# ChaissonLab/LRA

Hardware: AMD Instinct MI355X
Metric: aligned Gbp/s, 30 kb ONT vs GRCh38 (MapRead_lowacc end to end incl. SAM text), per job (higher is better)
Workload: dtype int32

## Files before the change

lra_amd/csrc/merge_extend.hip:

```cpp
#include "common.h"
#include "scan.h"
#include "std_sort.h"
#include <rocprim/rocprim.hpp>

namespace {

struct MeArgs {
  uint64_t n_slots; int numAln; int K;
  const uint32_t* nChains; const uint64_t* chainStart; const uint32_t* nSplit; const uint32_t* spStatus; const uint8_t* spStrand; const int32_t* spChrom;
  const uint64_t* matchOff; const uint32_t* mq; const uint32_t* mt; const uint32_t* box;
  const uint64_t* pos;
  uint32_t* nCl; uint32_t* nGr; const uint64_t* clBase; const uint64_t* grBase;
  uint64_t* cStart; uint64_t* cEnd; int* cStrand; int* cChrom; int* cRead; uint32_t* cGroup;
  uint32_t* gFirst; uint32_t* gLast; uint32_t* gSlot;
  const uint32_t* eCount; uint32_t* gSize; const uint64_t* anchorOff;
  const uint32_t* eq; const uint32_t* et; const int* el;
  uint32_t* aq; uint32_t* at; int32_t* alen; uint32_t* gbox; int32_t* gstrand; int32_t* gchrom; uint64_t* scratch;
};

template <int PASS>
__global__ void me_merge(MeArgs a) {
  const uint64_t s = (uint64_t)blockIdx.x * blockDim.x + threadIdx.x;
  if (s >= a.n_slots) return;
  const uint64_t r = s / a.numAln;
  uint32_t nsp = 0;
  if ((uint32_t)(s % a.numAln) < a.nChains[r] && !a.spStatus[s]) nsp = a.nSplit[s];
  if (PASS == 0) { a.nCl[s] = nsp; a.nGr[s] = 0; }
  if (nsp == 0) return;
  const uint64_t cs = a.chainStart[s];
  const uint64_t cb = PASS ? a.clBase[s] : 0, gb = PASS ? a.grBase[s] : 0;
  uint32_t g = 0, g0 = 0;
  for (uint32_t t = 0; t < nsp; t++) {
    const uint64_t x = cs + t;
    if (t > 0) {
      const uint64_t xp = x - 1;
      int qdist = 9999, tdist = 9999;
      if (a.spChrom[xp] == a.spChrom[x] && a.spStrand[xp] == a.spStrand[x]) {
        const uint32_t pqs = a.box[4 * xp], pts = a.box[4 * xp + 2], pte = a.box[4 * xp + 3];
        const uint32_t cqe = a.box[4 * x + 1], cts = a.box[4 * x + 2], cte = a.box[4 * x + 3];
        qdist = pqs > cqe ? (int)(pqs - cqe) : 0;
        if (a.spStrand[xp] == 0) tdist = pts >= cte ? (int)(pts - cte) : 9999;
        else tdist = pte <= cts ? (int)(cts - pte) : 9999;
      }
      if (!(qdist <= 500 && tdist <= 500)) {
        if (PASS) { a.gFirst[gb + g] = (uint32_t)(cb + g0); a.gLast[gb + g] = (uint32_t)(cb + t - 1); a.gSlot[gb + g] = (uint32_t)s; }
        g++; g0 = t;
      }
    }
    if (PASS) {
      const uint64_t c = cb + t;
      a.cStart[c] = a.matchOff[x]; a.cEnd[c] = a.matchOff[x + 1]; a.cStrand[c] = a.spStrand[x]; a.cChrom[c] = a.spChrom[x]; a.cRead[c] = (int)r;
      a.cGroup[c] = (uint32_t)(gb + g);
    }
  }
  if (PASS) { a.gFirst[gb + g] = (uint32_t)(cb + g0); a.gLast[gb + g] = (uint32_t)(cb + nsp - 1); a.gSlot[gb + g] = (uint32_t)s; }
  g++;
  if (PASS == 0) a.nGr[s] = g;
}

__global__ void __launch_bounds__(64) me_keys(uint64_t ncl, const uint64_t* __restrict__ cStart, const uint64_t* __restrict__ cEnd, const uint32_t* __restrict__ mq,
                                              const uint32_t* __restrict__ mt, uint64_t* key, uint32_t* val) {
  for (uint64_t c = blockIdx.x; c < ncl; c += gridDim.x)
    for (uint64_t i = cStart[c] + threadIdx.x; i < cEnd[c]; i += 64) {
      const uint32_t q = mq[i], t = mt[i];
      key[i] = ((uint64_t)((long long)q - (long long)t + (1LL << 32)) << 31) | q;
      val[i] = (uint32_t)i;
    }
}

__global__ void __launch_bounds__(64) me_gather_sorted(uint64_t ncl, const uint64_t* __restrict__ cStart, const uint64_t* __restrict__ cEnd, const int* __restrict__ cChrom,
                                                       const uint64_t* __restrict__ pos, const uint32_t* __restrict__ val, const uint32_t* __restrict__ mq,
                                                       const uint32_t* __restrict__ mt, uint32_t* sq, uint32_t* st) {
  for (uint64_t c = blockIdx.x; c < ncl; c += gridDim.x) {
    const uint32_t coff = (uint32_t)pos[cChrom[c]];
    for (uint64_t i = cStart[c] + threadIdx.x; i < cEnd[c]; i += 64) { const uint32_t v = val[i]; sq[i] = mq[v]; st[i] = mt[v] + coff; }
  }
}

__global__ void me_group_size(uint64_t ng, MeArgs a) {
  const uint64_t g = (uint64_t)blockIdx.x * blockDim.x + threadIdx.x;
  if (g >= ng) return;
  uint32_t n = 0;
  for (uint32_t c = a.gFirst[g]; c <= a.gLast[g]; c++) n += a.eCount[c];
  a.gSize[g] = n;
}

__global__ void __launch_bounds__(64) me_concat(uint64_t ng, MeArgs a) {
  const int lane = threadIdx.x;
  for (uint64_t g = blockIdx.x; g < ng; g += gridDim.x) {
    uint64_t o = a.anchorOff[g];
    uint32_t qS = 0xFFFFFFFFu, qE = 0, tS = 0xFFFFFFFFu, tE = 0;
    for (uint32_t c = a.gFirst[g]; c <= a.gLast[g]; c++) {
      const uint64_t b = a.cStart[c];
      const uint32_t n = a.eCount[c];
      const uint32_t coff = (uint32_t)a.pos[a.cChrom[c]];
      for (uint32_t i = lane; i < n; i += 64) {
        const uint32_t q = a.eq[b + i], t = a.et[b + i] - coff; const int l = a.el[b + i];
        a.aq[o + i] = q; a.at[o + i] = t; a.alen[o + i] = l;
        qS = min(qS, q); qE = max(qE, q + (uint32_t)l); tS = min(tS, t); tE = max(tE, t + (uint32_t)l);
      }
      o += n;
    }
    for (int off = 32; off > 0; off >>= 1) {
      qS = min(qS, (uint32_t)__shfl_xor(qS, off)); qE = max(qE, (uint32_t)__shfl_xor(qE, off));
      tS = min(tS, (uint32_t)__shfl_xor(tS, off)); tE = max(tE, (uint32_t)__shfl_xor(tE, off));
    }
    if (lane == 0) {
      const bool any = o > a.anchorOff[g];
      a.gbox[4 * g] = any ? qS : 0; a.gbox[4 * g + 1] = any ? qE : 0; a.gbox[4 * g + 2] = any ? tS : 0; a.gbox[4 * g + 3] = any ? tE : 0;
      a.gstrand[g] = any ? a.cStrand[a.gLast[g]] : 0; a.gchrom[g] = any ? a.cChrom[a.gLast[g]] : 0;
    }
  }
}

struct LongLess {
  const uint32_t* Q; const uint32_t* T; const int32_t* L; int strand;
  __device__ bool operator()(uint64_t i, uint64_t j) const {
    if (strand == 0) { if (Q[i] != Q[j]) return Q[i] < Q[j]; return T[i] < T[j]; }
    const uint32_t ei = Q[i] + (uint32_t)L[i], ej = Q[j] + (uint32_t)L[j];
    if (ei != ej) return ei > ej;
    return T[i] < T[j];
  }
};

__global__ void me_trim(uint64_t ng, const uint64_t* __restrict__ anchorOff, uint32_t* aq, uint32_t* at, int32_t* alen, const int32_t* __restrict__ gstrand,
                        uint64_t* scratch, int minLen) {
  const uint64_t g = (uint64_t)blockIdx.x * blockDim.x + threadIdx.x;
  if (g >= ng) return;
  const uint64_t b = anchorOff[g];
  const uint32_t n = (uint32_t)(anchorOff[g + 1] - b);
  uint32_t* Q = aq + b; uint32_t* T = at + b; int32_t* L = alen + b;
  uint64_t* idx = scratch + b;
  const int S = gstrand ? gstrand[g] : 0;
  uint32_t m = 0;
  for (uint32_t i = 0; i < n; i++) if (L[i] >= minLen) idx[m++] = i;
  LongLess lt{Q, T, L, S};
  lra_std_sort::std_sort(idx, (long)m, lt);
  for (uint32_t ln = 1; ln < m; ln++) {
    const uint32_t prev = (uint32_t)idx[ln - 1], cur = (uint32_t)idx[ln];
    int overlap_r = 0, overlap_g = 0;
    if (S == 0) {
      if (Q[cur] < Q[prev] + (uint32_t)L[prev] && Q[cur] >= Q[prev] + (uint32_t)L[prev] - 30u) overlap_r = (int)(Q[prev] + (uint32_t)L[prev] - Q[cur]);
    } else {
      if (Q[cur] + (uint32_t)L[cur] > Q[prev] && Q[cur] + (uint32_t)L[cur] <= Q[prev] + 30u) overlap_r = (int)(Q[cur] + (uint32_t)L[cur] - Q[prev]);
    }
    if (T[cur] < T[prev] + (uint32_t)L[prev] && T[cur] >= T[prev] + (uint32_t)L[prev] - 30u) overlap_g = (int)(T[prev] + (uint32_t)L[prev] - T[cur]);
    if (overlap_r > 0 || overlap_g > 0) {
      const int overlap = max(overlap_r, overlap_g);
      if (S == 1) Q[prev] += (uint32_t)(overlap + 1);
      L[prev] -= overlap + 1;
    }
  }
}

__global__ void me_iota(uint64_t n, uint64_t* out) {
  const uint64_t i = (uint64_t)blockIdx.x * blockDim.x + threadIdx.x;
  if (i <= n) out[i] = i;
}

__global__ void me_gather_off(uint64_t n, const uint64_t* idx, const uint64_t* src, uint64_t* out) {
  const uint64_t i = (uint64_t)blockIdx.x * blockDim.x + threadIdx.x;
  if (i <= n) out[i] = src[idx[i]];
}

inline size_t sz(size_t n, size_t e) { return (n * e + 255) / 256 * 256; }

}

extern "C" int lra_merge_extend_batch(lra_ctx* ctx, const lra_chain_result* ch, const lra_split_result* sp, const lra_btwn_result* bt, const char* d_seq,
                                      const uint64_t* d_read_off, const char* d_genome, const uint64_t* h_chrom_pos, int n_chrom, int K,
                                      lra_merge_result* out) {
  if (!ctx || !ch || !sp || !bt || !out || !h_chrom_pos || n_chrom < 1 || K < 1) return LRA_ERR_INVALID;
  memset(out, 0, sizeof *out);
  LRA_HIP_CHECK(ctx, hipSetDevice(ctx->device));
  hipStream_t st = ctx->stream;
  const uint64_t slots = sp->n_slots, NM = bt->n_matches;
  out->n_slots = slots;
  if (slots == 0) return LRA_OK;
  const size_t npos = (size_t)n_chrom + 1;
  auto take = [](char*& p, size_t n, size_t e) { char* r = p; p += sz(n, e); return r; };
  char* w = (char*)lra_ensure(ctx, 37, sz(slots + 2, 4) * 2 + sz(slots + 2, 8) * 2 + sz(npos, 8) + 4096);
  if (!w) return LRA_ERR_NOMEM;
  MeArgs a;
  memset(&a, 0, sizeof a);
  a.n_slots = slots; a.numAln = ch->num_aln; a.K = K; a.nChains = ch->d_n_chains; a.chainStart = ch->d_chain_start; a.nSplit = sp->d_n_split; a.spStatus = sp->d_status;
  a.spStrand = sp->d_sp_strand; a.spChrom = sp->d_sp_chrom; a.matchOff = bt->d_match_off; a.mq = bt->d_match_q; a.mt = bt->d_match_t; a.box = bt->d_box;
  a.nCl = (uint32_t*)take(w, slots + 2, 4); a.nGr = (uint32_t*)take(w, slots + 2, 4);
  uint64_t* clBase = (uint64_t*)take(w, slots + 2, 8); uint64_t* grBase = (uint64_t*)take(w, slots + 2, 8);
  uint64_t* dpos = (uint64_t*)take(w, npos, 8);
  a.clBase = clBase; a.grBase = grBase; a.pos = dpos;
  LRA_HIP_CHECK(ctx, hipMemcpyAsync(dpos, h_chrom_pos, npos * 8, hipMemcpyHostToDevice, st));
  const unsigned gs = (unsigned)((slots + 255) / 256);
  lra_time_begin(ctx, "merge_extend");
  hipLaunchKernelGGL(me_merge<0>, dim3(gs), dim3(256), 0, st, a);
  lra_time_end(ctx);
  { int rc = lra_exclusive_scan<uint32_t>(ctx, (long)slots, a.nCl, clBase); if (rc) return rc; }
  { int rc = lra_exclusive_scan<uint32_t>(ctx, (long)slots, a.nGr, grBase); if (rc) return rc; }
  uint64_t NCL = 0, NG = 0;
  LRA_HIP_CHECK(ctx, hipMemcpyAsync(&NCL, clBase + slots, 8, hipMemcpyDeviceToHost, st));
  LRA_HIP_CHECK(ctx, hipMemcpyAsync(&NG, grBase + slots, 8, hipMemcpyDeviceToHost, st));
  LRA_HIP_CHECK(ctx, hipStreamSynchronize(st));
  out->n_groups = NG; out->d_slot_group_off = grBase;
  char* wc = (char*)lra_ensure(ctx, 38, sz(NCL + 1, 8) * 2 + sz(NCL + 1, 4) * 5 + sz(4 * NCL + 4, 4) + sz(NG + 2, 4) * 6 + sz(4 * NG + 4, 4) + sz(NG + 2, 8) * 2 + 4096);
  char* wm = (char*)lra_ensure(ctx, 100, sz(NM + 1, 8) * 2 + sz(NM + 1, 4) * 6 + 4096);
  if (!wc || !wm) return LRA_ERR_NOMEM;
  a.cStart = (uint64_t*)take(wc, NCL + 1, 8); a.cEnd = (uint64_t*)take(wc, NCL + 1, 8);
  a.cStrand = (int*)take(wc, NCL + 1, 4); a.cChrom = (int*)take(wc, NCL + 1, 4); a.cRead = (int*)take(wc, NCL + 1, 4); a.cGroup = (uint32_t*)take(wc, NCL + 1, 4);
  uint32_t* eCount = (uint32_t*)take(wc, NCL + 1, 4); uint32_t* ebox = (uint32_t*)take(wc, 4 * NCL + 4, 4);
  a.gFirst = (uint32_t*)take(wc, NG + 2, 4); a.gLast = (uint32_t*)take(wc, NG + 2, 4); a.gSlot = (uint32_t*)take(wc, NG + 2, 4); a.gSize = (uint32_t*)take(wc, NG + 2, 4);
  a.gstrand = (int32_t*)take(wc, NG + 2, 4); a.gchrom = (int32_t*)take(wc, NG + 2, 4); a.gbox = (uint32_t*)take(wc, 4 * NG + 4, 4);
  uint64_t* anchorOff = (uint64_t*)take(wc, NG + 2, 8); uint64_t* iota = (uint64_t*)take(wc, NG + 2, 8);
  uint64_t* key = (uint64_t*)take(wm, NM + 1, 8); uint64_t* key2 = (uint64_t*)take(wm, NM + 1, 8);
  uint32_t* val = (uint32_t*)take(wm, NM + 1, 4); uint32_t* val2 = (uint32_t*)take(wm, NM + 1, 4); uint32_t* sq = (uint32_t*)take(wm, NM + 1, 4);
  uint32_t* stt = (uint32_t*)take(wm, NM + 1, 4); uint32_t* eq = (uint32_t*)take(wm, NM + 1, 4); uint32_t* et = (uint32_t*)take(wm, NM + 1, 4);
  int* el = (int*)key;
  a.eCount = eCount; a.eq = eq; a.et = et; a.el = el; a.anchorOff = anchorOff; a.scratch = key2;
  if (NCL == 0) { LRA_HIP_CHECK(ctx, hipMemsetAsync(anchorOff, 0, 16, st)); LRA_HIP_CHECK(ctx, hipStreamSynchronize(st)); out->d_anchor_off = anchorOff; return LRA_OK; }
  lra_time_begin(ctx, "merge_extend");
  hipLaunchKernelGGL(me_merge<1>, dim3(gs), dim3(256), 0, st, a);
  lra_time_end(ctx);
  const unsigned gw = (unsigned)std::min<uint64_t>(NCL, (uint64_t)ctx->num_cu * 32);
  if (NM > 0) {
    lra_time_begin(ctx, "merge_extend");
    hipLaunchKernelGGL(me_keys, dim3(gw), dim3(64), 0, st, NCL, (const uint64_t*)a.cStart, (const uint64_t*)a.cEnd, a.mq, a.mt, key, val);
    const int rc = lra_segsort_pairs_scratch(ctx, key, key2, val, val2, NM, NCL, a.cStart, a.cEnd, 0, 64);
    if (rc) { lra_time_end(ctx); return rc; }
    hipLaunchKernelGGL(me_gather_sorted, dim3(gw), dim3(64), 0, st, NCL, (const uint64_t*)a.cStart, (const uint64_t*)a.cEnd, (const int*)a.cChrom, (const uint64_t*)dpos,
                       (const uint32_t*)val2, a.mq, a.mt, sq, stt);
    lra_time_end(ctx);
  }
  { int rc = lra_launch_linear_extend(ctx, NCL, K, a.cStart, a.cEnd, a.cStrand, a.cChrom, a.cRead, sq, stt, dpos, (const unsigned char*)d_genome,
                                      (const unsigned char*)d_seq, d_read_off, eq, et, el, eCount, ebox); if (rc) return rc; }
  lra_time_begin(ctx, "merge_extend");
  hipLaunchKernelGGL(me_group_size, dim3((unsigned)((NG + 255) / 256)), dim3(256), 0, st, NG, a);
  lra_time_end(ctx);
  { int rc = lra_exclusive_scan<uint32_t>(ctx, (long)NG, a.gSize, anchorOff); if (rc) return rc; }
  uint64_t NA = 0;
  LRA_HIP_CHECK(ctx, hipMemcpyAsync(&NA, anchorOff + NG, 8, hipMemcpyDeviceToHost, st));
  LRA_HIP_CHECK(ctx, hipStreamSynchronize(st));
  char* wa = (char*)lra_ensure(ctx, 39, sz(NA + 1, 4) * 3 + 1024);
  if (!wa) return LRA_ERR_NOMEM;
  a.aq = (uint32_t*)take(wa, NA + 1, 4); a.at = (uint32_t*)take(wa, NA + 1, 4); a.alen = (int32_t*)take(wa, NA + 1, 4);
  lra_time_begin(ctx, "merge_extend");
  hipLaunchKernelGGL(me_concat, dim3((unsigned)std::min<uint64_t>(NG, (uint64_t)ctx->num_cu * 32)), dim3(64), 0, st, NG, a);
  hipLaunchKernelGGL(me_trim, dim3((unsigned)((NG + 63) / 64)), dim3(64), 0, st, NG, (const uint64_t*)anchorOff, a.aq, a.at, a.alen, (const int32_t*)a.gstrand, a.scratch, 40);
  hipLaunchKernelGGL(me_iota, dim3((unsigned)((NG + 256) / 256)), dim3(256), 0, st, NG, iota);
  lra_time_end(ctx);
  LRA_HIP_CHECK(ctx, hipStreamSynchronize(st));
  LRA_HIP_CHECK(ctx, hipGetLastError());
  out->n_anchors = NA; out->d_anchor_off = anchorOff; out->d_count = a.gSize; out->d_q = a.aq; out->d_t = a.at; out->d_len = a.alen; out->d_box = a.gbox;
  out->d_strand = a.gstrand; out->d_chrom = a.gchrom; out->d_group_slot = a.gSlot; out->d_group_first = a.gFirst; out->d_group_last = a.gLast; out->d_cluster_base = clBase;
  out->d_iota = iota;
  return LRA_OK;
}

extern "C" int lra_trim_anchor_pairs_batch(lra_ctx* ctx, uint64_t n_lists, const uint64_t* d_off, uint64_t n_anchors, uint32_t* d_q, uint32_t* d_t, int32_t* d_len) {
  if (!ctx) return LRA_ERR_INVALID;
  if (n_lists == 0 || n_anchors == 0) return LRA_OK;
  LRA_HIP_CHECK(ctx, hipSetDevice(ctx->device));
  uint64_t* scratch = (uint64_t*)lra_scratch(ctx, 2, (n_anchors + 1) * 8);
  if (!scratch) return LRA_ERR_NOMEM;
  lra_time_begin(ctx, "merge_extend");
  hipLaunchKernelGGL(me_trim, dim3((unsigned)((n_lists + 63) / 64)), dim3(64), 0, ctx->stream, n_lists, d_off, d_q, d_t, d_len, (const int32_t*)nullptr, scratch, 50);
  lra_time_end(ctx);
  LRA_HIP_CHECK(ctx, hipStreamSynchronize(ctx->stream));
  LRA_HIP_CHECK(ctx, hipGetLastError());
  return LRA_OK;
}

extern "C" int lra_trim_overlapped_anchors_batch(lra_ctx* ctx, uint64_t n_clusters, const uint64_t* d_off, uint64_t n_anchors, const int32_t* d_strand,
                                                 uint32_t* d_q, uint32_t* d_t, int32_t* d_len) {
  if (!ctx || (n_clusters && !d_strand)) return LRA_ERR_INVALID;
  if (n_clusters == 0 || n_anchors == 0) return LRA_OK;
  LRA_HIP_CHECK(ctx, hipSetDevice(ctx->device));
  uint64_t* scratch = (uint64_t*)lra_scratch(ctx, 2, (n_anchors + 1) * 8);
  if (!scratch) return LRA_ERR_NOMEM;
  lra_time_begin(ctx, "merge_extend");
  hipLaunchKernelGGL(me_trim, dim3((unsigned)((n_clusters + 63) / 64)), dim3(64), 0, ctx->stream, n_clusters, d_off, d_q, d_t, d_len, d_strand, scratch, 40);
  lra_time_end(ctx);
  LRA_HIP_CHECK(ctx, hipStreamSynchronize(ctx->stream));
  LRA_HIP_CHECK(ctx, hipGetLastError());
  return LRA_OK;
}

namespace {
struct SdArgs {
  uint64_t n_clusters;
  const uint64_t* a_off; const uint32_t* q; const uint32_t* t; const int32_t* len; const uint8_t* overlap; const int32_t* strand;
  int merge_dist;
  uint32_t* cnt; const uint64_t* g_off; uint32_t* g_start; uint32_t* g_end; uint32_t* status;
};
__device__ __forceinline__ bool sd_head(const SdArgs& a, uint64_t base, long i, int strand) {
  const uint64_t x = base + i, p = x - 1;
  const long dq = strand == 0 ? (long)a.t[x] - (long)a.q[x] : (long)a.q[x] + (long)a.t[x] + a.len[x];
  const long dp = strand == 0 ? (long)a.t[p] - (long)a.q[p] : (long)a.q[p] + (long)a.t[p] + a.len[p];
  const uint32_t prevEnd = a.q[p] + (uint32_t)a.len[p];
  const long gap = labs((long)a.q[x] - ((long)a.q[p] + a.len[p]));
  return !(a.overlap[p] == 0 && a.overlap[x] == 0 && dp == dq && prevEnd < a.q[x] && gap <= a.merge_dist);
}
template <bool EMIT>
__global__ void __launch_bounds__(64) sd_kernel(SdArgs a) {
  const uint64_t c = blockIdx.x;
  const int lane = threadIdx.x;
  if (c >= a.n_clusters) return;
  const uint64_t base = a.a_off[c];
  const long n = (long)(a.a_off[c + 1] - base);
  if (n <= 0) { if (!EMIT && lane == 0) { a.cnt[c] = 0; a.status[c] = LRA_ST_OOB_SLOT; } return; }
  const int strand = a.strand[c];
  const unsigned long long below = (lane == 0) ? 0ULL : (~0ULL >> (64 - lane));
  uint32_t ng = 0;
  const uint64_t go = EMIT ? a.g_off[c] : 0;
  for (long i0 = 0; i0 < n; i0 += 64) {
    const long i = i0 + lane;
    const bool head = i < n && (i == 0 || sd_head(a, base, i, strand));
    const unsigned long long m = __ballot(head);
    if (EMIT && head) {
      const uint32_t g = ng + (uint32_t)__popcll(m & below);
      a.g_start[go + g] = (uint32_t)i;
      if (g > 0) a.g_end[go + g - 1] = (uint32_t)i;
    }
    ng += (uint32_t)__popcll(m);
  }
  if (lane == 0) {
    if (EMIT) a.g_end[go + ng - 1] = (uint32_t)n;
    else { a.cnt[c] = ng; a.status[c] = 0; }
  }
}
}

extern "C" int lra_merge_same_diag_batch(lra_ctx* ctx, uint64_t n_clusters, const uint64_t* d_anchor_off, const uint32_t* d_q, const uint32_t* d_t,
                                         const int32_t* d_len, const uint8_t* d_overlap, const int32_t* d_strand, int merge_dist,
                                         lra_same_diag_result* out) {
  if (!ctx || !out) return LRA_ERR_INVALID;
  memset(out, 0, sizeof *out);
  out->n_clusters = n_clusters;
  if (n_clusters == 0) return LRA_OK;
  LRA_HIP_CHECK(ctx, hipSetDevice(ctx->device));
  hipStream_t st = ctx->stream;
  const size_t n1 = (size_t)n_clusters + 2;
  char* w = (char*)lra_ensure(ctx, 67, ((n1 * 4 + 255) & ~(size_t)255) * 2 + ((n1 * 8 + 255) & ~(size_t)255) + 4096);
  if (!w) return LRA_ERR_NOMEM;
  uint32_t* cnt = (uint32_t*)w; w += (n1 * 4 + 255) & ~(size_t)255;
  uint32_t* status = (uint32_t*)w; w += (n1 * 4 + 255) & ~(size_t)255;
  uint64_t* g_off = (uint64_t*)w;
  SdArgs a; memset(&a, 0, sizeof a);
  a.n_clusters = n_clusters; a.a_off = d_anchor_off; a.q = d_q; a.t = d_t; a.len = d_len; a.overlap = d_overlap; a.strand = d_strand; a.merge_dist = merge_dist;
  a.cnt = cnt; a.status = status;
  lra_time_begin(ctx, "merge_same_diag");
  hipLaunchKernelGGL(sd_kernel<false>, dim3((unsigned)n_clusters), dim3(64), 0, st, a);
  lra_time_end(ctx);
  { int rc = lra_exclusive_scan<uint32_t>(ctx, (long)n_clusters, cnt, g_off); if (rc) return rc; }
  uint64_t ng = 0;
  LRA_HIP_CHECK(ctx, hipMemcpyAsync(&ng, g_off + n_clusters, 8, hipMemcpyDeviceToHost, st));
  LRA_HIP_CHECK(ctx, hipStreamSynchronize(st));
  uint32_t* gs = (uint32_t*)lra_ensure(ctx, 68, (ng + 1) * 8 + 512);
  if (!gs) return LRA_ERR_NOMEM;
  uint32_t* ge = gs + ((ng + 64) & ~(uint64_t)63);
  a.g_off = g_off; a.g_start = gs; a.g_end = ge;
  lra_time_begin(ctx, "merge_same_diag");
  hipLaunchKernelGGL(sd_kernel<true>, dim3((unsigned)n_clusters), dim3(64), 0, st, a);
  lra_time_end(ctx);
  LRA_HIP_CHECK(ctx, hipStreamSynchronize(st));
  LRA_HIP_CHECK(ctx, hipGetLastError());
  out->n_groups = ng; out->d_group_off = g_off; out->d_start = gs; out->d_end = ge; out->d_status = status;
  return LRA_OK;
}


namespace {
struct SoArgs {
  uint64_t n_elems;
  const int32_t* e_cluster; const uint32_t* e_entry; const uint64_t* g_off; const uint32_t* start; const uint32_t* end; const int32_t* coarse;
  uint32_t* cnt; const uint64_t* out_off; uint32_t* out_anchor; int32_t* out_cluster;
};
__global__ void so_count(SoArgs a) {
  const uint64_t i = (uint64_t)blockIdx.x * blockDim.x + threadIdx.x;
  if (i >= a.n_elems) return;
  const uint64_t g = a.g_off[a.e_cluster[i]] + a.e_entry[i];
  a.cnt[i] = a.end[g] > a.start[g] ? a.end[g] - a.start[g] : 0u;
}
__global__ void __launch_bounds__(64) so_emit(SoArgs a) {
  const uint64_t i = blockIdx.x;
  if (i >= a.n_elems) return;
  const int c = a.e_cluster[i];
  const uint64_t g = a.g_off[c] + a.e_entry[i];
  const uint32_t s = a.start[g], e = a.end[g];
  const uint64_t o = a.out_off[i];
  const int co = a.coarse[c];
  for (uint32_t x = threadIdx.x; s + x < e; x += 64) { a.out_anchor[o + x] = e - 1 - x; a.out_cluster[o + x] = co; }
}
}

extern "C" int lra_switch_to_original_anchors_batch(lra_ctx* ctx, uint64_t n_chains, const uint64_t* d_chain_off, uint64_t n_elems, const int32_t* d_elem_cluster,
                                                    const uint32_t* d_elem_entry, const lra_same_diag_result* same_diag, const int32_t* d_coarse,
                                                    lra_original_anchors_result* out) {
  if (!ctx || !out || !same_diag) return LRA_ERR_INVALID;
  memset(out, 0, sizeof *out);
  out->n_chains = n_chains;
  if (n_chains == 0 || n_elems == 0) return LRA_OK;
  LRA_HIP_CHECK(ctx, hipSetDevice(ctx->device));
  hipStream_t st = ctx->stream;
  auto al = [](size_t x) { return (x + 255) & ~(size_t)255; };
  char* w = (char*)lra_ensure(ctx, 76, al((n_elems + 2) * 4) + al((n_elems + 2) * 8) + al((n_chains + 2) * 8) + 4096);
  if (!w) return LRA_ERR_NOMEM;
  SoArgs a; memset(&a, 0, sizeof a);
  a.n_elems = n_elems; a.e_cluster = d_elem_cluster; a.e_entry = d_elem_entry; a.g_off = same_diag->d_group_off; a.start = same_diag->d_start; a.end = same_diag->d_end;
  a.coarse = d_coarse;
  a.cnt = (uint32_t*)w; w += al((n_elems + 2) * 4);
  uint64_t* e_off = (uint64_t*)w; w += al((n_elems + 2) * 8);
  uint64_t* c_off = (uint64_t*)w;
  hipLaunchKernelGGL(so_count, dim3((unsigned)((n_elems + 255) / 256)), dim3(256), 0, st, a);
  { int rc = lra_exclusive_scan<uint32_t>(ctx, (long)n_elems, a.cnt, e_off); if (rc) return rc; }
  uint64_t total = 0;
  LRA_HIP_CHECK(ctx, hipMemcpyAsync(&total, e_off + n_elems, 8, hipMemcpyDeviceToHost, st));
  LRA_HIP_CHECK(ctx, hipStreamSynchronize(st));
  uint32_t* oa = (uint32_t*)lra_ensure(ctx, 77, al((total + 1) * 4) * 2 + 512);
  if (!oa) return LRA_ERR_NOMEM;
  int32_t* oc = (int32_t*)((char*)oa + al((total + 1) * 4));
  a.out_off = e_off; a.out_anchor = oa; a.out_cluster = oc;
  hipLaunchKernelGGL(so_emit, dim3((unsigned)n_elems), dim3(64), 0, st, a);
  hipLaunchKernelGGL(me_gather_off, dim3((unsigned)((n_chains + 256) / 256)), dim3(256), 0, st, n_chains, d_chain_off, (const uint64_t*)e_off, c_off);
  LRA_HIP_CHECK(ctx, hipStreamSynchronize(st));
  LRA_HIP_CHECK(ctx, hipGetLastError());
  out->n_anchors = total; out->d_chain_off = c_off; out->d_anchor = oa; out->d_cluster = oc;
  return LRA_OK;
}
```

lra_amd/csrc/refine_btwn.hip:

```cpp
#include "common.h"
#include "scan.h"
#include <rocprim/rocprim.hpp>
#include <algorithm>
#include <vector>

namespace {

constexpr uint32_t NONE = 0xFFFFFFFFu;

struct Seg { uint64_t off; uint32_t len; uint32_t next; };

struct BtArgs {
  uint64_t n_slots; int numAln;
  const uint32_t* nChains; const uint64_t* chainStart; const uint32_t* nSplit; const uint32_t* spStatus; const uint8_t* spStrand; const int32_t* spChrom;
  const uint8_t* splitLink;
  const uint64_t* read_off; uint64_t rcBase;
  const uint64_t* pos; int npos;
  int K, W; uint32_t RSD; float sparse2;
  int round;
  uint32_t* box; uint32_t* cnt; uint8_t* rspace; uint32_t* segHead; uint32_t* segTail;
  uint32_t* need; const uint64_t* needOff;
  uint64_t* pQoff; int32_t* pQlen; uint64_t* pToff; int32_t* pTlen; uint32_t* pTspan; int32_t* pK; int32_t* pW; int32_t* pDiag; uint32_t* pQadd;
  uint32_t* pTadd; uint32_t* pFlip;
  uint32_t* mSpan; uint8_t* mKind; uint8_t* mTwo; uint8_t* mSt; uint32_t* mX; uint32_t* mXp;
  const uint64_t* pairOff; const uint64_t* pool; uint64_t poolU, poolS;
  Seg* segs; uint32_t* segCount; uint32_t segCap; uint32_t* overflow;
};

__device__ __forceinline__ int space_diag(uint32_t qe, uint32_t qs) {
  return min((int)floorf(fmaxf(100.f, 0.15f * (float)(qe - qs))), 1000);
}

__device__ void plan_problem(const BtArgs& a, uint64_t s, int j, uint64_t r, uint32_t readLen, int chrom, uint32_t qe, uint32_t qs, uint32_t te, uint32_t ts,
                             int st, uint32_t lrts, uint32_t lrlength, int kind, int two, uint32_t x, uint32_t xp) {
  if (st == 1) { const uint32_t t = qs; qs = readLen - qe; qe = readLen - t; }
  const uint64_t i = 2 * s + j;
  a.need[i] = 1;
  a.pQoff[i] = (st ? a.rcBase : 0) + a.read_off[r] + qs; a.pQlen[i] = (int32_t)(qe - qs);
  a.pToff[i] = a.pos[chrom] + (ts - lrts); a.pTlen[i] = (int32_t)(te - ts + lrlength); a.pTspan[i] = te - (ts - lrts);
  a.pK[i] = a.K; a.pW[i] = a.W; a.pDiag[i] = space_diag(qe, qs); a.pQadd[i] = qs; a.pTadd[i] = ts - lrts; a.pFlip[i] = st == 1 ? readLen : 0;
  a.mSpan[i] = min(qe - qs, te - ts); a.mKind[i] = (uint8_t)kind; a.mTwo[i] = (uint8_t)two; a.mSt[i] = (uint8_t)st; a.mX[i] = x; a.mXp[i] = xp;
}

__global__ void bt_plan(BtArgs a) {
  const uint64_t s = (uint64_t)blockIdx.x * blockDim.x + threadIdx.x;
  if (s >= a.n_slots) return;
  a.need[2 * s] = 0; a.need[2 * s + 1] = 0;
  const uint64_t r = s / a.numAln;
  if ((uint32_t)(s % a.numAln) >= a.nChains[r] || a.spStatus[s]) return;
  const uint32_t nsp = a.nSplit[s];
  const uint64_t cs = a.chainStart[s];
  const uint32_t readLen = (uint32_t)(a.read_off[r + 1] - a.read_off[r]);
  auto glen = [&](int c) { return a.pos[c + 1] - a.pos[c]; };
  if (a.round >= 1) {
    const uint32_t c = (uint32_t)a.round;
    if (c >= nsp) return;
    const uint64_t xc = cs + c, xp = cs + c - 1;
    if (a.cnt[xc] == 0 || a.cnt[xp] == 0) return;
    const uint32_t cqs = a.box[4 * xc], cqe = a.box[4 * xc + 1], cts = a.box[4 * xc + 2], cte = a.box[4 * xc + 3];
    const uint32_t pqs = a.box[4 * xp], pts = a.box[4 * xp + 2], pte = a.box[4 * xp + 3];
    (void)cqs;
    const int cst = a.spStrand[xc], pst = a.spStrand[xp], link = a.splitLink[cs + c - 1];
    const int cchrom = a.spChrom[xc], pchrom = a.spChrom[xp];
    const uint32_t qs = cqe, qe = pqs;
    uint32_t ts1 = 0, te1 = 0, ts2 = 0, te2 = 0;
    if (qe <= qs) return;
    const uint32_t gap = qe - qs;
    int st1 = 0, st2 = 0, two = 0;
    if (cst == pst && link == 0) {
      two = 0; st1 = cst;
      if (cte <= pts) { ts1 = cte; te1 = pts; }
      else if (cts > pte) { ts1 = pte; te1 = cts; }
      else return;
    } else if (cst != pst && link == 1) {
      st1 = cst; st2 = pst; two = 1;
      if (cte <= pts) {
        if (st1 == 0) { ts1 = cte; te1 = ts1 + gap; ts2 = pte; te2 = ts2 + gap; }
        else { te1 = cts; ts1 = te1 > gap ? te1 - gap : 0; te2 = pts; ts2 = te2 > gap ? te2 - gap : 0; }
      } else if (cts > pte) {
        if (st1 == 0) { ts1 = cte; te1 = ts1 + gap; te2 = cts; ts2 = te2 > gap ? te2 - gap : 0; }
        else { te1 = cts; ts1 = te1 > gap ? te1 - gap : 0; te2 = pts; ts2 = te2 > gap ? te2 - gap : 0; }
      } else return;
    } else if (cst == pst && link == 1) {
      st1 = cst; st2 = st1; two = 1;
      if (st1 == 0 && cte > pts) { ts1 = cte; te1 = ts1 + gap; te2 = pts; ts2 = te2 > gap ? te2 - gap : 0; }
      else if (st1 == 1 && cts < pte) { te1 = cts; ts1 = te1 > gap ? te1 - gap : 0; ts2 = pte; te2 = ts2 + gap; }
      else return;
    }
    if (te1 <= ts1) return;
    if (te1 >= glen(cchrom)) return;
    if (max(gap, te1 - ts1) >= 5 * a.RSD) return;
    uint32_t space = max(gap, te1 - ts1);
    if (space >= 20 && space <= a.RSD && cchrom == pchrom)
      plan_problem(a, s, 0, r, readLen, cchrom, qe, qs, te1, ts1, st1, 0, 0, 0, two, (uint32_t)(xc - cs), (uint32_t)(xp - cs));
    if (two) {
      if (te2 <= ts2) return;
      if (te2 >= glen(cchrom)) return;
      if (max(gap, te2 - ts2) >= 5 * a.RSD) return;
      space = max(gap, te2 - ts2);
      if (space >= 20 && space <= a.RSD && cchrom == pchrom)
        plan_problem(a, s, 1, r, readLen, pchrom, qe, qs, te2, ts2, st2, 0, 0, 1, 1, (uint32_t)(xp - cs), (uint32_t)(xp - cs));
    }
    return;
  }
  if (nsp == 0) return;
  if (a.round == -1) {
    const uint64_t x = cs;
    if (a.cnt[x] == 0) return;
    const int st = a.spStrand[x], chrom = a.spChrom[x];
    const uint32_t qs = a.box[4 * x + 1], qe = readLen;
    uint32_t ts = 0, te = 0;
    if (st == 0) { ts = a.box[4 * x + 3]; te = ts + qe - qs; }
    else { te = a.box[4 * x + 2]; if (te > qe - qs) ts = te - (qe - qs); else return; }
    if (!(qe > qs && te > ts)) return;
    const uint32_t space = max(qe - qs, te - ts);
    if (!(space >= 20 && space < a.RSD && (uint64_t)te + 500 < glen(chrom))) return;
    uint32_t lrts = 0, lrlength = 0;
    if (st == 0) { lrts = 0; lrlength = 500; } else { if (ts > 500) lrts = 500; lrlength = lrts; }
    plan_problem(a, s, 0, r, readLen, chrom, qe, qs, te, ts, st, lrts, lrlength, 1, 1, 0, 0);
  } else {
    const uint64_t x = cs + nsp - 1;
    if (a.cnt[x] == 0) return;
    const int st = a.spStrand[x], chrom = a.spChrom[x];
    const uint32_t qs = 0, qe = a.box[4 * x];
    uint32_t ts, te;
    if (st == 0) { te = a.box[4 * x + 2]; ts = te > qe - qs ? te - (qe - qs) : 0; }
    else { ts = a.box[4 * x + 3]; te = ts + (qe - qs); }
    if (!(qe > qs && te > ts)) return;
    const uint32_t space = max(qe - qs, te - ts);
    if (!(space >= 20 && space < a.RSD && (uint64_t)te + 500 < glen(chrom))) return;
    uint32_t lrts = 0, lrlength = 0;
    if (st == 0) { if (ts > 500) lrts = 500; lrlength = lrts; } else { lrts = 0; lrlength = 500; }
    plan_problem(a, s, 0, r, readLen, chrom, qe, qs, te, ts, st, lrts, lrlength, 1, 1, nsp - 1, nsp - 1);
  }
}

__global__ void bt_compact(BtArgs a, uint64_t* dQoff, int32_t* dQlen, uint64_t* dToff, int32_t* dTlen, uint32_t* dTspan, int32_t* dK, int32_t* dW,
                           int32_t* dDiag, uint32_t* dQadd, uint32_t* dTadd, uint32_t* dFlip) {
  const uint64_t i = (uint64_t)blockIdx.x * blockDim.x + threadIdx.x;
  if (i >= 2 * a.n_slots || !a.need[i]) return;
  const uint64_t p = a.needOff[i];
  dQoff[p] = a.pQoff[i]; dQlen[p] = a.pQlen[i]; dToff[p] = a.pToff[i]; dTlen[p] = a.pTlen[i]; dTspan[p] = a.pTspan[i]; dK[p] = a.pK[i]; dW[p] = a.pW[i];
  dDiag[p] = a.pDiag[i]; dQadd[p] = a.pQadd[i]; dTadd[p] = a.pTadd[i]; dFlip[p] = a.pFlip[i];
}

__global__ void bt_pack(uint64_t n, const uint32_t* __restrict__ q, const uint32_t* __restrict__ t, uint64_t* out) {
  const uint64_t i = (uint64_t)blockIdx.x * blockDim.x + threadIdx.x;
  if (i < n) out[i] = ((uint64_t)q[i] << 32) | t[i];
}

__device__ void append_seg(const BtArgs& a, uint64_t x, uint64_t off, uint32_t len) {
  if (len == 0) return;
  const uint32_t id = atomicAdd(a.segCount, 1u);
  if (id >= a.segCap) { *a.overflow = 1; return; }
  a.segs[id].off = off; a.segs[id].len = len; a.segs[id].next = NONE;
  if (a.segHead[x] == NONE) a.segHead[x] = id; else a.segs[a.segTail[x]].next = id;
  a.segTail[x] = id;
  uint32_t qs = a.box[4 * x], qe = a.box[4 * x + 1], ts = a.box[4 * x + 2], te = a.box[4 * x + 3];
  for (uint32_t i = 0; i < len; i++) {
    const uint64_t v = a.pool[off + i];
    const uint32_t q = (uint32_t)(v >> 32), t = (uint32_t)v;
    qs = min(qs, q); qe = max(qe, q + (uint32_t)a.K); ts = min(ts, t); te = max(te, t + (uint32_t)a.K);
  }
  a.box[4 * x] = qs; a.box[4 * x + 1] = qe; a.box[4 * x + 2] = ts; a.box[4 * x + 3] = te;
  a.cnt[x] += len;
}

__global__ void bt_apply(BtArgs a) {
  const uint64_t s = (uint64_t)blockIdx.x * blockDim.x + threadIdx.x;
  if (s >= a.n_slots) return;
  for (int j = 0; j < 2; j++) {
    const uint64_t i = 2 * s + j;
    if (!a.need[i]) continue;
    const uint64_t cs = a.chainStart[s];
    const uint64_t p = a.needOff[i];
    const uint64_t p0 = a.pairOff[p];
    const uint32_t n = (uint32_t)(a.pairOff[p + 1] - p0);
    const float eff = ((float)n) / (float)a.mSpan[i];
    const uint64_t x = cs + a.mX[i], xp = cs + a.mXp[i];
    if (n == 0) continue;
    if (a.mKind[i] == 1) { append_seg(a, x, a.poolU + p0, n); a.rspace[x] = 1; continue; }
    if (eff >= a.sparse2) { append_seg(a, x, a.poolU + p0, n); a.rspace[x] = 1; continue; }
    if (a.mTwo[i]) continue;
    const uint64_t* S = a.pool + a.poolS + p0;
    const int st = a.mSt[i];
    uint32_t start = 0;
    while (start < n) {
      uint32_t end = start + 1;
      while (end < n) {
        const long long dq = llabs((long long)(uint32_t)(S[end] >> 32) - (long long)(uint32_t)(S[end - 1] >> 32));
        const long long dt = llabs((long long)(uint32_t)S[end] - (long long)(uint32_t)S[end - 1]);
        if (min(dq, dt) <= 200) end++; else break;
      }
      if (end - start >= 4) {
        uint32_t qS = (uint32_t)(S[start] >> 32), qE = qS + a.K, tS = (uint32_t)S[start], tE = tS + a.K;
        for (uint32_t k = start + 1; k < end; k++) {
          const uint32_t q = (uint32_t)(S[k] >> 32), t = (uint32_t)S[k];
          tE = max(tE, t + (uint32_t)a.K); tS = min(tS, t); qE = max(qE, q + (uint32_t)a.K); qS = min(qS, q);
        }
        const uint32_t cqe = a.box[4 * x + 1], cts = a.box[4 * x + 2], cte = a.box[4 * x + 3];
        const uint32_t pqs = a.box[4 * xp], pts = a.box[4 * xp + 2], pte = a.box[4 * xp + 3];
        int qd = qS >= cqe ? (int)(qS - cqe) : 0, td;
        if (st == 0) td = tS >= cte ? (int)(tS - cte) : 0; else td = cts >= tE ? (int)(cts - tE) : 0;
        const int dist_cur = max(qd, td);
        qd = pqs >= qE ? (int)(pqs - qE) : 0;
        if (st == 0) td = pts >= tE ? (int)(pts - tE) : 0; else td = tS >= pte ? (int)(tS - pte) : 0;
        const int dist_prev = max(qd, td);
        append_seg(a, dist_cur <= dist_prev ? x : xp, a.poolS + p0 + start, end - start);
      }
      start = end;
    }
  }
}

struct LayArgs {
  uint64_t n_slots; int numAln; int K;
  const uint32_t* nChains; const uint64_t* chainStart; const uint32_t* nSplit; const uint32_t* spStatus;
  const uint64_t* baseOff; const uint32_t* baseQ; const uint32_t* baseT;
  const uint32_t* cnt; const uint32_t* box; const uint32_t* segHead; const Seg* segs; const uint64_t* pool;
  const uint64_t* outOff; uint32_t* oq; uint32_t* ot; float* eff;
};

__global__ void __launch_bounds__(64) bt_layout(LayArgs a) {
  const uint64_t s = blockIdx.x;
  const uint64_t r = s / a.numAln;
  if ((uint32_t)(s % a.numAln) >= a.nChains[r] || a.spStatus[s]) return;
  const uint64_t cs = a.chainStart[s];
  const int lane = threadIdx.x;
  for (uint32_t k = 0; k < a.nSplit[s]; k++) {
    const uint64_t x = cs + k;
    uint64_t o = a.outOff[x];
    const uint64_t b0 = a.baseOff[x], b1 = a.baseOff[x + 1];
    for (uint64_t i = b0 + lane; i < b1; i += 64) { a.oq[o + (i - b0)] = a.baseQ[i]; a.ot[o + (i - b0)] = a.baseT[i]; }
    o += b1 - b0;
    for (uint32_t g = a.segHead[x]; g != NONE; g = a.segs[g].next) {
      const Seg sg = a.segs[g];
      for (uint32_t i = lane; i < sg.len; i += 64) { const uint64_t v = a.pool[sg.off + i]; a.oq[o + i] = (uint32_t)(v >> 32); a.ot[o + i] = (uint32_t)v; }
      o += sg.len;
    }
    if (lane == 0) {
      const uint32_t n = a.cnt[x];
      a.eff[x] = n ? ((float)n) / (float)min(a.box[4 * x + 1] - a.box[4 * x], a.box[4 * x + 3] - a.box[4 * x + 2]) : 0.f;
    }
  }
}

__global__ void bt_init(uint64_t nf, const uint64_t* __restrict__ baseOff, const uint32_t* __restrict__ baseBox, uint32_t* cnt, uint32_t* box,
                        uint32_t* segHead, uint32_t* segTail, uint8_t* rspace) {
  const uint64_t x = (uint64_t)blockIdx.x * blockDim.x + threadIdx.x;
  if (x > nf) return;
  if (x == nf) { cnt[x] = 0; return; }
  cnt[x] = (uint32_t)(baseOff[x + 1] - baseOff[x]);
  box[4 * x] = baseBox[4 * x]; box[4 * x + 1] = baseBox[4 * x + 1]; box[4 * x + 2] = baseBox[4 * x + 2]; box[4 * x + 3] = baseBox[4 * x + 3];
  segHead[x] = NONE; segTail[x] = NONE; rspace[x] = 0;
}

inline size_t sz(size_t n, size_t e) { return (n * e + 255) / 256 * 256; }

void* grow_keep(lra_ctx* ctx, int slot, size_t used, size_t need) {
  if (ctx->gbuf[slot] && ctx->gbytes[slot] >= need) return ctx->gbuf[slot];
  const size_t want = need + need / 2 + 4096;
  void* p = nullptr;
  if (hipMalloc(&p, want) != hipSuccess) { lra_set_err(ctx, LRA_ERR_NOMEM, "hipMalloc(%zu) failed", want); return nullptr; }
  if (ctx->gbuf[slot]) {
    if (used) (void)hipMemcpyAsync(p, ctx->gbuf[slot], used, hipMemcpyDeviceToDevice, ctx->stream);
    (void)hipStreamSynchronize(ctx->stream);
    (void)hipFree(ctx->gbuf[slot]);
  }
  ctx->gbuf[slot] = p; ctx->gbytes[slot] = want;
  return p;
}

}

extern "C" int lra_refine_btwn_splitchain_batch(lra_ctx* ctx, const lra_chain_result* ch, const lra_split_result* sp, const lra_refined_result* rf,
                                                const uint64_t* d_read_off, const char* d_strands, uint64_t rc_base, const char* d_genome,
                                                const uint64_t* h_chrom_pos, int n_chrom, const lra_btwn_opts* opts, lra_btwn_result* out) {
  if (!ctx || !ch || !sp || !rf || !out || !opts || !h_chrom_pos || n_chrom < 1) return LRA_ERR_INVALID;
  memset(out, 0, sizeof *out);
  LRA_HIP_CHECK(ctx, hipSetDevice(ctx->device));
  hipStream_t st = ctx->stream;
  const uint64_t slots = sp->n_slots, NF = sp->n_frags;
  out->n_frags = NF;
  if (slots == 0) return LRA_OK;
  const size_t npos = (size_t)n_chrom + 1, n2 = 2 * slots;
  auto take = [](char*& p, size_t n, size_t e) { char* r = p; p += sz(n, e); return r; };
  char* w = (char*)lra_ensure(ctx, 35, sz(NF + 2, 4) * 3 + sz(4 * NF + 4, 4) + sz(NF + 2, 1) + sz(NF + 2, 8) + sz(NF + 1, 4) + sz(npos, 8) + sz(n2 + 1, 4) * 12 +
                                           sz(n2 + 2, 8) * 3 + sz(n2 + 1, 1) * 3 + 4096);
  if (!w) return LRA_ERR_NOMEM;
  BtArgs a;
  memset(&a, 0, sizeof a);
  a.n_slots = slots; a.numAln = ch->num_aln; a.nChains = ch->d_n_chains; a.chainStart = ch->d_chain_start; a.nSplit = sp->d_n_split; a.spStatus = sp->d_status;
  a.spStrand = sp->d_sp_strand; a.spChrom = sp->d_sp_chrom; a.splitLink = sp->d_split_link; a.read_off = d_read_off; a.rcBase = rc_base;
  a.K = opts->K; a.W = opts->W; a.RSD = (uint32_t)opts->refineSpaceDist; a.sparse2 = opts->anchorstoosparse * 2;
  a.cnt = (uint32_t*)take(w, NF + 2, 4); a.segHead = (uint32_t*)take(w, NF + 2, 4); a.segTail = (uint32_t*)take(w, NF + 2, 4);
  a.box = (uint32_t*)take(w, 4 * NF + 4, 4); a.rspace = (uint8_t*)take(w, NF + 2, 1);
  uint64_t* outOff = (uint64_t*)take(w, NF + 2, 8); float* eff = (float*)take(w, NF + 1, 4);
  uint64_t* dpos = (uint64_t*)take(w, npos, 8);
  a.pos = dpos; a.npos = (int)npos;
  a.need = (uint32_t*)take(w, n2 + 1, 4); a.pQlen = (int32_t*)take(w, n2 + 1, 4); a.pTlen = (int32_t*)take(w, n2 + 1, 4); a.pTspan = (uint32_t*)take(w, n2 + 1, 4);
  a.pK = (int32_t*)take(w, n2 + 1, 4); a.pW = (int32_t*)take(w, n2 + 1, 4); a.pDiag = (int32_t*)take(w, n2 + 1, 4); a.pQadd = (uint32_t*)take(w, n2 + 1, 4);
  a.pTadd = (uint32_t*)take(w, n2 + 1, 4); a.pFlip = (uint32_t*)take(w, n2 + 1, 4); a.mSpan = (uint32_t*)take(w, n2 + 1, 4); a.mX = (uint32_t*)take(w, n2 + 1, 4);
  uint64_t* needOff = (uint64_t*)take(w, n2 + 2, 8); a.pQoff = (uint64_t*)take(w, n2 + 2, 8); a.pToff = (uint64_t*)take(w, n2 + 2, 8);
  a.mKind = (uint8_t*)take(w, n2 + 1, 1); a.mTwo = (uint8_t*)take(w, n2 + 1, 1); a.mSt = (uint8_t*)take(w, n2 + 1, 1);
  a.needOff = needOff;
  char* wd = (char*)lra_ensure(ctx, 36, sz(n2 + 1, 4) * 10 + sz(n2 + 1, 8) * 2 + 4096);
  if (!wd) return LRA_ERR_NOMEM;
  a.mXp = (uint32_t*)take(wd, n2 + 1, 4);
  uint64_t* dQoff = (uint64_t*)take(wd, n2 + 1, 8); uint64_t* dToff = (uint64_t*)take(wd, n2 + 1, 8);
  int32_t* dQlen = (int32_t*)take(wd, n2 + 1, 4); int32_t* dTlen = (int32_t*)take(wd, n2 + 1, 4); uint32_t* dTspan = (uint32_t*)take(wd, n2 + 1, 4);
  int32_t* dK = (int32_t*)take(wd, n2 + 1, 4); int32_t* dW = (int32_t*)take(wd, n2 + 1, 4); int32_t* dDiag = (int32_t*)take(wd, n2 + 1, 4);
  uint32_t* dQadd = (uint32_t*)take(wd, n2 + 1, 4); uint32_t* dTadd = (uint32_t*)take(wd, n2 + 1, 4); uint32_t* dFlip = (uint32_t*)take(wd, n2 + 1, 4);
  LRA_HIP_CHECK(ctx, hipMemcpyAsync(dpos, h_chrom_pos, npos * 8, hipMemcpyHostToDevice, st));
  hipLaunchKernelGGL(bt_init, dim3((unsigned)((NF + 256) / 256)), dim3(256), 0, st, NF, rf->d_match_off, rf->d_box, a.cnt, a.box, a.segHead, a.segTail, a.rspace);
  std::vector<uint32_t> h_nsplit(slots);
  LRA_HIP_CHECK(ctx, hipMemcpyAsync(h_nsplit.data(), sp->d_n_split, slots * 4, hipMemcpyDeviceToHost, st));
  LRA_HIP_CHECK(ctx, hipStreamSynchronize(st));
  uint32_t maxSplit = 0;
  for (uint64_t i = 0; i < slots; i++) maxSplit = std::max(maxSplit, h_nsplit[i]);
  const int SEG_SLOT = 32, POOL_SLOT = 33, OUT_SLOT = 34;
  uint32_t* segCtl = (uint32_t*)lra_scratch(ctx, 3, 256);
  if (!segCtl) return LRA_ERR_NOMEM;
  LRA_HIP_CHECK(ctx, hipMemsetAsync(segCtl, 0, 256, st));
  a.segCount = segCtl; a.overflow = segCtl + 1;
  uint64_t poolUsed = 0; uint32_t segUsedBound = 0;
  std::vector<int> rounds;
  for (uint32_t c = 1; c < maxSplit; c++) rounds.push_back((int)c);
  if (maxSplit > 0) { rounds.push_back(-1); rounds.push_back(-2); }
  const unsigned gs = (unsigned)((slots + 255) / 256), g2 = (unsigned)((n2 + 255) / 256);
  uint64_t totalProblems = 0, totalPairs = 0;
  for (int rd : rounds) {
    a.round = rd;
    lra_time_begin(ctx, "btwn_plan");
    hipLaunchKernelGGL(bt_plan, dim3(gs), dim3(256), 0, st, a);
    lra_time_end(ctx);
    { int rc = lra_exclusive_scan<uint32_t>(ctx, (long)n2, a.need, needOff); if (rc) return rc; }
    uint64_t np = 0;
    LRA_HIP_CHECK(ctx, hipMemcpyAsync(&np, needOff + n2, 8, hipMemcpyDeviceToHost, st));
    LRA_HIP_CHECK(ctx, hipStreamSynchronize(st));
    if (np == 0) continue;
    totalProblems += np;
    hipLaunchKernelGGL(bt_compact, dim3(g2), dim3(256), 0, st, a, dQoff, dQlen, dToff, dTlen, dTspan, dK, dW, dDiag, dQadd, dTadd, dFlip);
    lra_refine_space_result rs;
    { int rc = lra_refine_space_batch(ctx, (int)np, d_strands, dQoff, dQlen, d_genome, dToff, dTlen, dTspan, dK, dW, dDiag, dQadd, dTadd, dFlip, opts->match,
                                      opts->mismatch, opts->indel, opts->max_freq, &rs); if (rc) return rc; }
    const uint64_t nP = rs.n_pairs;
    totalPairs += nP;
    uint64_t* pool = (uint64_t*)grow_keep(ctx, POOL_SLOT, poolUsed * 8, (poolUsed + 2 * nP + 2) * 8);
    if (!pool) return LRA_ERR_NOMEM;
    const uint32_t segPrev = segUsedBound;
    segUsedBound += (uint32_t)(nP / 4 + 2 * np + 2);
    Seg* segs = (Seg*)grow_keep(ctx, SEG_SLOT, (size_t)segPrev * sizeof(Seg), (size_t)segUsedBound * sizeof(Seg));
    if (!segs) return LRA_ERR_NOMEM;
    a.pool = pool; a.poolU = poolUsed; a.poolS = poolUsed + nP; a.segs = segs; a.segCap = segUsedBound; a.pairOff = rs.d_pair_off;
    if (nP > 0) {
      lra_time_begin(ctx, "btwn_apply");
      hipLaunchKernelGGL(bt_pack, dim3((unsigned)((nP + 255) / 256)), dim3(256), 0, st, nP, rs.d_pair_q, rs.d_pair_t, pool + poolUsed);
      size_t temp_bytes = 0;
      (void)rocprim::segmented_radix_sort_keys(nullptr, temp_bytes, (uint64_t*)nullptr, (uint64_t*)nullptr, (unsigned int)nP, (unsigned int)np, (uint64_t*)nullptr,
                                               (uint64_t*)nullptr, 0, 64, st);
      void* temp = lra_scratch(ctx, 2, temp_bytes + 256);
      if (!temp) { lra_time_end(ctx); return LRA_ERR_NOMEM; }
      hipError_t e = rocprim::segmented_radix_sort_keys(temp, temp_bytes, pool + poolUsed, pool + poolUsed + nP, (unsigned int)nP, (unsigned int)np, rs.d_pair_off,
                                                        rs.d_pair_off + 1, 0, 64, st);
      lra_time_end(ctx);
      if (e != hipSuccess) return lra_set_err(ctx, LRA_ERR_HIP, "segmented sort: %s", hipGetErrorString(e));
    }
    lra_time_begin(ctx, "btwn_apply");
    hipLaunchKernelGGL(bt_apply, dim3(gs), dim3(256), 0, st, a);
    lra_time_end(ctx);
    poolUsed += 2 * nP;
  }
  uint32_t ctl[2] = {0, 0};
  LRA_HIP_CHECK(ctx, hipMemcpyAsync(ctl, segCtl, 8, hipMemcpyDeviceToHost, st));
  LRA_HIP_CHECK(ctx, hipStreamSynchronize(st));
  if (ctl[1]) return lra_set_err(ctx, LRA_ERR_HIP, "internal: segment pool overflow");
  { int rc = lra_exclusive_scan<uint32_t>(ctx, (long)NF + 1, a.cnt, outOff); if (rc) return rc; }
  uint64_t NM = 0;
  LRA_HIP_CHECK(ctx, hipMemcpyAsync(&NM, outOff + NF, 8, hipMemcpyDeviceToHost, st));
  LRA_HIP_CHECK(ctx, hipStreamSynchronize(st));
  char* wm = (char*)lra_ensure(ctx, OUT_SLOT, sz(NM + 1, 4) * 2 + 1024);
  if (!wm) return LRA_ERR_NOMEM;
  uint32_t* oq = (uint32_t*)take(wm, NM + 1, 4); uint32_t* ot = (uint32_t*)take(wm, NM + 1, 4);
  LayArgs l;
  memset(&l, 0, sizeof l);
  l.n_slots = slots; l.numAln = ch->num_aln; l.K = opts->K; l.nChains = ch->d_n_chains; l.chainStart = ch->d_chain_start; l.nSplit = sp->d_n_split; l.spStatus = sp->d_status;
  l.baseOff = rf->d_match_off; l.baseQ = rf->d_match_q; l.baseT = rf->d_match_t; l.cnt = a.cnt; l.box = a.box; l.segHead = a.segHead;
  l.segs = (const Seg*)ctx->gbuf[SEG_SLOT]; l.pool = (const uint64_t*)ctx->gbuf[POOL_SLOT]; l.outOff = outOff; l.oq = oq; l.ot = ot; l.eff = eff;
  lra_time_begin(ctx, "btwn_apply");
  hipLaunchKernelGGL(bt_layout, dim3((unsigned)slots), dim3(64), 0, st, l);
  lra_time_end(ctx);
  LRA_HIP_CHECK(ctx, hipStreamSynchronize(st));
  LRA_HIP_CHECK(ctx, hipGetLastError());
  out->n_matches = NM; out->n_problems = totalProblems; out->n_pairs = totalPairs; out->n_rounds = (uint32_t)rounds.size();
  out->d_match_off = outOff; out->d_match_q = oq; out->d_match_t = ot; out->d_box = a.box; out->d_eff = eff; out->d_refinespace = a.rspace;
  return LRA_OK;
}
```

lra_amd/csrc/refine_splitchain.hip:

```cpp
#include "common.h"
#include "append_values.h"
#include "scan.h"
#include <vector>

namespace {

struct RscArgs {
  uint64_t n_slots; int numAln;
  const uint32_t* nChains; const uint64_t* chainStart;
  const uint32_t* cq; const uint32_t* ct; const int32_t* clen; const uint32_t* ccl; const uint8_t* cstrand;
  const uint32_t* nSplit; const uint32_t* spBeg; const uint32_t* spLen; const uint32_t* spIdx; const uint8_t* spStrand; const int32_t* spChrom;
  const uint32_t* spBox; const uint32_t* ciBeg; const uint32_t* ciLen; const uint32_t* ciIdx; const uint32_t* fidx; const uint32_t* spStatus;
  const uint64_t* read_off;
  const uint64_t* pos; int npos;
  const uint64_t* qWinOff; const uint64_t* qBnd; uint64_t n_reads;
  const uint64_t* gSeqOff; uint64_t nWg; const uint64_t* gBnd;
  int window, smallK, K, limitrefine, lwin;
  uint32_t* taskCnt; const uint64_t* taskOff; uint32_t* status;
  uint64_t* qLo; uint64_t* qHi; uint64_t* tLo; uint64_t* tHi; uint32_t* qAdd; uint32_t* tAdd; int64_t* mx; int64_t* mn;
};

__device__ int header_find(const uint64_t* pos, int npos, uint64_t query, bool& ub) {
  if (npos > 0 && query == pos[0]) return 0;
  int lo = 0, cnt = npos;
  while (cnt > 0) { const int step = cnt >> 1; if (pos[lo + step] < query) { lo += step + 1; cnt -= step + 1; } else cnt = step; }
  if (lo == npos) { ub = true; return lo - 1; }
  if (query == pos[lo]) return lo;
  return lo - 1;
}

__device__ long lookup_index(const uint64_t* so, long n, uint64_t pos, bool& ub) {
  if (n == 0) return 0;
  long lo = 0, cnt = n;
  while (cnt > 0) { const long step = cnt >> 1; if (so[lo + step] < pos) { lo += step + 1; cnt -= step + 1; } else cnt = step; }
  if (lo == n) { ub = true; return lo - 1; }
  if (so[lo] != pos) return lo - 1;
  return lo;
}

template <bool EMIT>
__global__ void __launch_bounds__(64) rsc_tasks(RscArgs a) {
  const uint64_t s = (uint64_t)blockIdx.x * blockDim.x + threadIdx.x;
  if (s >= a.n_slots) return;
  const uint64_t r = s / a.numAln;
  if ((uint32_t)(s % a.numAln) >= a.nChains[r]) return;
  const uint64_t cs = a.chainStart[s];
  const uint32_t readLen = (uint32_t)(a.read_off[r + 1] - a.read_off[r]);
  const long nWq = ((long)readLen + a.lwin - 1) / a.lwin;
  const uint32_t nsp = a.spStatus[s] ? 0 : a.nSplit[s];
  for (uint32_t k = 0; k < nsp; k++) {
    const uint64_t x = cs + k;
    const int m = (int)a.spLen[x];
    uint32_t ntask = 0;
    uint64_t to = EMIT ? a.taskOff[x] : 0;
    if (!EMIT) { a.taskCnt[x] = 0; a.status[x] = 0; }
    else if (a.status[x]) continue;
    if (m == 0) continue;
    const uint32_t* idx = a.spIdx + cs + a.spBeg[x];
    const uint32_t* ci = a.ciIdx + cs + a.ciBeg[x];
    const int nci = (int)a.ciLen[x];
    const int Strand = a.spStrand[x];
    const uint32_t chromOffset = (uint32_t)a.pos[a.spChrom[x]];
    auto flipped = [&](uint32_t c) { for (int j = 0; j < nci; j++) if (ci[j] == c) return true; return false; };
    auto AN = [&](int i) { return cs + a.fidx[cs + idx[i]]; };
    auto tS = [&](int i) { const uint64_t p = AN(i); return flipped(a.ccl[p]) ? a.ct[p] - chromOffset : a.ct[p]; };
    auto qS = [&](int i) { const uint64_t p = AN(i); return (a.cstrand[p] == 1 && flipped(a.ccl[p])) ? readLen - (a.cq[p] + (uint32_t)a.K) : a.cq[p]; };
    auto qE = [&](int i) { return qS(i) + (uint32_t)a.clen[AN(i)]; };
    const uint32_t QStart = a.spBox[4 * x], QEnd = a.spBox[4 * x + 1], TStart = a.spBox[4 * x + 2], TEnd = a.spBox[4 * x + 3];
    bool ub = false;
    const int fi = header_find(a.pos, a.npos, TEnd, ub);
    if (ub || fi + 1 >= a.npos) { if (!EMIT) a.status[x] = LRA_ST_OOB_SLOT; continue; }
    const uint32_t chromEndOffset = (uint32_t)a.pos[fi + 1];
    int64_t maxDN = (int64_t)tS(0) - (int64_t)qS(0), minDN = maxDN;
    if (!a.limitrefine)
      for (int db = 0; db < m; db++) { const int64_t d = (int64_t)tS(db) - (int64_t)qS(db); maxDN = max(maxDN, d); minDN = min(minDN, d); }
    const int64_t maxDiagNum = maxDN + 50, minDiagNum = minDN - 50;
    const uint32_t wts = (TStart >= chromOffset + (uint32_t)a.window) ? TStart - a.window : chromOffset;
    const uint32_t wte = (TEnd + (uint32_t)a.window < chromEndOffset) ? TEnd + a.window : chromEndOffset;
    const long ls = lookup_index(a.gSeqOff, (long)a.nWg + 1, wts, ub), le = lookup_index(a.gSeqOff, (long)a.nWg + 1, wte, ub);
    if (ub) { if (!EMIT) a.status[x] = LRA_ST_OOB_SLOT; continue; }
    const uint32_t qStart = Strand == 0 ? QStart : readLen - QEnd, qEnd = Strand == 0 ? QEnd : readLen - QStart;
    const uint64_t w0 = a.qWinOff[(Strand ? a.n_reads : 0) + r];
    int matchStart = 0, matchEnd = 0;
    bool bad = false;
    for (long lsi = ls; lsi <= le && !bad; lsi++) {
      if (lsi + 1 > (long)a.nWg) continue;
      if (a.gSeqOff[lsi] < chromOffset || a.gSeqOff[lsi + 1] < chromOffset) continue;
      const uint32_t gStart = (uint32_t)(a.gSeqOff[lsi] - chromOffset), gEnd = (uint32_t)(a.gSeqOff[lsi + 1] - 1 - chromOffset);
      if (gStart >= gEnd) continue;
      while (matchStart < m && tS(matchStart) <= gStart) matchStart++;
      matchEnd = matchStart;
      while (matchEnd < m && tS(matchEnd) < gEnd) matchEnd++;
      if (matchStart >= m) continue;
      if (matchEnd == matchStart) continue;
      uint32_t readStart = qS(matchStart), readEnd = qS(matchEnd - 1);
      int64_t miniMin = (int64_t)tS(matchStart) - (int64_t)qS(matchStart);
      const int64_t miniMax = (int64_t)1 << 60;
      for (int mi = matchStart; mi < matchEnd; mi++) {
        const uint32_t q0 = qS(mi), q1 = q0 + (uint32_t)a.clen[AN(mi)];
        if (q0 < readStart) readStart = q0;
        if (q1 > readEnd) readEnd = q1;
        const int64_t d = (int64_t)tS(mi) - (int64_t)q0;
        miniMin = min(miniMin, d);
      }
      if (readStart == readEnd) { if (lsi > ls && readStart > 0) readStart = 0; }
      miniMin -= 100;
      const uint32_t sow = 500;
      if (lsi == ls) readStart = (readStart < sow) ? 0 : readStart - sow;
      if (lsi == le) readEnd = (readEnd + sow > readLen) ? readLen : readEnd + sow;
      if (readStart > readEnd) continue;
      const uint32_t e2 = min(readEnd, readLen - 1);
      const long qi0 = readStart == readLen ? nWq : (long)(readStart / (uint32_t)a.lwin);
      const long qi1 = (long)(e2 / (uint32_t)a.lwin);
      if (readStart > readLen) { bad = true; break; }
      for (long qi = qi0; qi <= qi1; ++qi) {
        if (EMIT) {
          a.qLo[to] = a.qBnd[w0 + qi]; a.qHi[to] = a.qBnd[w0 + qi + 1];
          a.tLo[to] = a.gBnd[lsi]; a.tHi[to] = a.gBnd[lsi + 1];
          a.qAdd[to] = (uint32_t)min((long)readLen, qi * (long)a.lwin); a.tAdd[to] = gStart;
          a.mx[to] = a.limitrefine ? miniMax : maxDiagNum; a.mn[to] = a.limitrefine ? miniMin : minDiagNum;
          to++;
        }
        ntask++;
      }
    }
    (void)qE; (void)qStart; (void)qEnd;
    if (bad) { if (!EMIT) { a.status[x] = LRA_ST_OOB_SLOT; a.taskCnt[x] = 0; } continue; }
    if (!EMIT) a.taskCnt[x] = ntask;
  }
}

typedef AvArgs FilterArgs;

__global__ void rsc_task_box(uint64_t n_slots, int numAln, const uint32_t* nChains, const uint64_t* chainStart, const uint32_t* nSplit,
                             const uint32_t* spStatus, const uint64_t* taskOff, const uint32_t* spBox, const uint8_t* spStrand, const int32_t* spChrom,
                             const uint64_t* pos, const uint64_t* read_off, uint32_t* tbox) {
  const uint64_t s = (uint64_t)blockIdx.x;
  const uint64_t r = s / numAln;
  if ((uint32_t)(s % numAln) >= nChains[r] || spStatus[s]) return;
  const uint64_t cs = chainStart[s];
  const uint32_t readLen = (uint32_t)(read_off[r + 1] - read_off[r]);
  for (uint32_t k = 0; k < nSplit[s]; k++) {
    const uint64_t x = cs + k;
    const uint32_t chromOffset = (uint32_t)pos[spChrom[x]];
    const uint32_t QStart = spBox[4 * x], QEnd = spBox[4 * x + 1], TStart = spBox[4 * x + 2], TEnd = spBox[4 * x + 3];
    const int st = spStrand[x];
    const uint32_t qs = st == 0 ? QStart : readLen - QEnd, qe = st == 0 ? QEnd : readLen - QStart;
    for (uint64_t t = taskOff[x] + threadIdx.x; t < taskOff[x + 1]; t += blockDim.x) {
      tbox[4 * t] = qs; tbox[4 * t + 1] = qe; tbox[4 * t + 2] = TStart - chromOffset; tbox[4 * t + 3] = TEnd - chromOffset;
    }
  }
}

struct FinishArgs {
  uint64_t n_slots; int numAln; int smallK;
  const uint32_t* nChains; const uint64_t* chainStart; const uint32_t* nSplit; const uint32_t* spStatus; const uint8_t* spStrand;
  const uint64_t* taskOff; const uint64_t* outOff; const uint64_t* read_off;
  uint64_t* matchOff; uint32_t* oq; const uint32_t* ot; uint32_t* box; float* eff; uint64_t nf;
};

__global__ void rsc_match_off(FinishArgs a) {
  const uint64_t x = (uint64_t)blockIdx.x * blockDim.x + threadIdx.x;
  if (x > a.nf) return;
  a.matchOff[x] = a.outOff[a.taskOff[x]];
}

__global__ void __launch_bounds__(64) rsc_finish(FinishArgs a) {
  const uint64_t s = blockIdx.x;
  const uint64_t r = s / a.numAln;
  if ((uint32_t)(s % a.numAln) >= a.nChains[r] || a.spStatus[s]) return;
  const uint64_t cs = a.chainStart[s];
  const uint32_t readLen = (uint32_t)(a.read_off[r + 1] - a.read_off[r]);
  const int lane = threadIdx.x;
  for (uint32_t k = 0; k < a.nSplit[s]; k++) {
    const uint64_t x = cs + k;
    const uint64_t m0 = a.matchOff[x], m1 = a.matchOff[x + 1];
    if (m1 == m0) { if (lane == 0) { a.box[4 * x] = 0; a.box[4 * x + 1] = 0; a.box[4 * x + 2] = 0; a.box[4 * x + 3] = 0; a.eff[x] = 0; } continue; }
    const bool rev = a.spStrand[x] == 1;
    uint32_t qmin = 0xFFFFFFFFu, qmax = 0, tmin = 0xFFFFFFFFu, tmax = 0;
    for (uint64_t i = m0 + lane; i < m1; i += 64) {
      uint32_t q = a.oq[i];
      if (rev) { q = readLen - (q + (uint32_t)a.smallK); a.oq[i] = q; }
      const uint32_t t = a.ot[i];
      qmin = min(qmin, q); qmax = max(qmax, q + (uint32_t)a.smallK); tmin = min(tmin, t); tmax = max(tmax, t + (uint32_t)a.smallK);
    }
    for (int o = 32; o > 0; o >>= 1) {
      qmin = min(qmin, __shfl_xor(qmin, o)); qmax = max(qmax, __shfl_xor(qmax, o));
      tmin = min(tmin, __shfl_xor(tmin, o)); tmax = max(tmax, __shfl_xor(tmax, o));
    }
    if (lane == 0) {
      a.box[4 * x] = qmin; a.box[4 * x + 1] = qmax; a.box[4 * x + 2] = tmin; a.box[4 * x + 3] = tmax;
      a.eff[x] = ((float)(m1 - m0)) / (float)min(qmax - qmin, tmax - tmin);
    }
  }
}

inline size_t sz(size_t n, size_t e) { return (n * e + 255) / 256 * 256; }

}

extern "C" int lra_refine_splitchain_batch(lra_ctx* ctx, const lra_chain_result* ch, const lra_split_result* sp, const uint64_t* d_read_off,
                                           const uint64_t* h_chrom_pos, int n_chrom, const lra_local_index_result* read_index,
                                           uint64_t n_g_windows, const uint64_t* d_g_seq_off, const uint64_t* d_g_tuple_bnd,
                                           const uint32_t* d_g_tuples, const lra_rsc_opts* opts, lra_refined_result* out) {
  if (!ctx || !ch || !sp || !out || !opts || !h_chrom_pos || n_chrom < 1 || !read_index) return LRA_ERR_INVALID;
  if (opts->local_window <= 0) return lra_set_err(ctx, LRA_ERR_INVALID, "local_window must be positive");
  if (read_index->n_seqs != 2 * ch->n_reads) return lra_set_err(ctx, LRA_ERR_INVALID, "read_index must hold the reads forward, then reverse-complemented");
  memset(out, 0, sizeof *out);
  LRA_HIP_CHECK(ctx, hipSetDevice(ctx->device));
  hipStream_t st = ctx->stream;
  const uint64_t slots = sp->n_slots, NF = sp->n_frags;
  out->n_frags = NF;
  if (slots == 0) return LRA_OK;
  const size_t npos = (size_t)n_chrom + 1;
  auto take = [](char*& p, size_t n, size_t e) { char* r = p; p += sz(n, e); return r; };
  char* w = (char*)lra_ensure(ctx, 27, sz(NF + 2, 4) * 2 + sz(NF + 2, 8) * 2 + sz(4 * NF + 4, 4) + sz(NF + 1, 4) + sz(npos, 8) + 4096);
  if (!w) return LRA_ERR_NOMEM;
  RscArgs a;
  memset(&a, 0, sizeof a);
  a.n_slots = slots; a.numAln = ch->num_aln; a.nChains = ch->d_n_chains; a.chainStart = ch->d_chain_start;
  a.cq = ch->d_chain_q; a.ct = ch->d_chain_t; a.clen = ch->d_chain_alen; a.ccl = ch->d_chain_cluster; a.cstrand = ch->d_chain_strand;
  a.nSplit = sp->d_n_split; a.spBeg = sp->d_sp_beg; a.spLen = sp->d_sp_len; a.spIdx = sp->d_sp_idx; a.spStrand = sp->d_sp_strand; a.spChrom = sp->d_sp_chrom;
  a.spBox = sp->d_sp_box; a.ciBeg = sp->d_ci_beg; a.ciLen = sp->d_ci_len; a.ciIdx = sp->d_ci_idx; a.fidx = sp->d_fidx; a.spStatus = sp->d_status;
  a.read_off = d_read_off;
  a.qWinOff = read_index->d_win_off; a.qBnd = read_index->d_tuple_bnd; a.n_reads = (uint64_t)ch->n_reads;
  a.gSeqOff = d_g_seq_off; a.nWg = n_g_windows; a.gBnd = d_g_tuple_bnd;
  a.window = opts->window; a.smallK = opts->smallK; a.K = opts->K; a.limitrefine = opts->limitrefine; a.lwin = opts->local_window;
  a.taskCnt = (uint32_t*)take(w, NF + 2, 4); a.status = (uint32_t*)take(w, NF + 2, 4);
  uint64_t* taskOff = (uint64_t*)take(w, NF + 2, 8); uint64_t* matchOff = (uint64_t*)take(w, NF + 2, 8);
  uint32_t* box = (uint32_t*)take(w, 4 * NF + 4, 4); float* eff = (float*)take(w, NF + 1, 4);
  uint64_t* dpos = (uint64_t*)take(w, npos, 8);
  a.pos = dpos; a.npos = (int)npos; a.taskOff = taskOff;
  LRA_HIP_CHECK(ctx, hipMemcpyAsync(dpos, h_chrom_pos, npos * 8, hipMemcpyHostToDevice, st));
  LRA_HIP_CHECK(ctx, hipMemsetAsync(a.taskCnt, 0, (NF + 2) * 4, st));
  LRA_HIP_CHECK(ctx, hipMemsetAsync(a.status, 0, (NF + 2) * 4, st));
  const unsigned gs = (unsigned)((slots + 63) / 64);
  lra_time_begin(ctx, "rsc_tasks");
  hipLaunchKernelGGL(rsc_tasks<false>, dim3(gs), dim3(64), 0, st, a);
  lra_time_end(ctx);
  { int rc = lra_exclusive_scan<uint32_t>(ctx, (long)NF + 1, a.taskCnt, taskOff); if (rc) return rc; }
  uint64_t NT = 0;
  LRA_HIP_CHECK(ctx, hipMemcpyAsync(&NT, taskOff + NF + 1, 8, hipMemcpyDeviceToHost, st));
  LRA_HIP_CHECK(ctx, hipStreamSynchronize(st));
  out->n_tasks = NT;
  out->d_match_off = matchOff; out->d_box = box; out->d_eff = eff; out->d_status = a.status;
  char* wt = (char*)lra_ensure(ctx, 28, sz(NT + 2, 8) * 7 + sz(NT + 1, 4) * 3 + sz(4 * NT + 4, 4) + 4096);
  if (!wt) return LRA_ERR_NOMEM;
  a.qLo = (uint64_t*)take(wt, NT + 2, 8); a.qHi = (uint64_t*)take(wt, NT + 2, 8); a.tLo = (uint64_t*)take(wt, NT + 2, 8); a.tHi = (uint64_t*)take(wt, NT + 2, 8);
  a.mx = (int64_t*)take(wt, NT + 2, 8); a.mn = (int64_t*)take(wt, NT + 2, 8); uint64_t* outOff = (uint64_t*)take(wt, NT + 2, 8);
  a.qAdd = (uint32_t*)take(wt, NT + 1, 4); a.tAdd = (uint32_t*)take(wt, NT + 1, 4);
  uint32_t* passCnt = (uint32_t*)take(wt, NT + 1, 4); uint32_t* tbox = (uint32_t*)take(wt, 4 * NT + 4, 4);
  FinishArgs f;
  memset(&f, 0, sizeof f);
  f.n_slots = slots; f.numAln = ch->num_aln; f.smallK = opts->smallK; f.nChains = ch->d_n_chains; f.chainStart = ch->d_chain_start; f.nSplit = sp->d_n_split;
  f.spStatus = sp->d_status; f.spStrand = sp->d_sp_strand; f.taskOff = taskOff; f.outOff = outOff; f.read_off = d_read_off; f.matchOff = matchOff;
  f.box = box; f.eff = eff; f.nf = NF;
  uint64_t NM = 0;
  uint32_t* oq = nullptr; uint32_t* ot = nullptr;
  if (NT > 0) {
    lra_time_begin(ctx, "rsc_tasks");
    hipLaunchKernelGGL(rsc_tasks<true>, dim3(gs), dim3(64), 0, st, a);
    hipLaunchKernelGGL(rsc_task_box, dim3((unsigned)slots), dim3(64), 0, st, slots, ch->num_aln, ch->d_n_chains, ch->d_chain_start, sp->d_n_split, sp->d_status,
                       (const uint64_t*)taskOff, sp->d_sp_box, sp->d_sp_strand, sp->d_sp_chrom, (const uint64_t*)dpos, d_read_off, tbox);
    lra_time_end(ctx);
    lra_local_pairs_result pr;
    { int rc = lra_local_compare_batch(ctx, NT, read_index->d_tuples, a.qLo, a.qHi, d_g_tuples, a.tLo, a.tHi, opts->max_freq, nullptr, nullptr, &pr); if (rc) return rc; }
    out->n_pairs = pr.n_pairs;
    FilterArgs fa;
    memset(&fa, 0, sizeof fa);
    fa.n_tasks = NT; fa.pairOff = pr.d_pair_off; fa.pqi = pr.d_pair_qi; fa.pti = pr.d_pair_ti; fa.qTup = read_index->d_tuples; fa.gTup = d_g_tuples;
    fa.qAdd = a.qAdd; fa.tAdd = a.tAdd; fa.mx = a.mx; fa.mn = a.mn; fa.tbox = tbox; fa.cnt = passCnt; fa.outOff = outOff;
    const unsigned gt = (unsigned)((NT + 63) / 64);
    lra_time_begin(ctx, "rsc_filter");
    hipLaunchKernelGGL(av_filter<false>, dim3(gt), dim3(64), 0, st, fa);
    lra_time_end(ctx);
    { int rc = lra_exclusive_scan<uint32_t>(ctx, (long)NT, passCnt, outOff); if (rc) return rc; }
    LRA_HIP_CHECK(ctx, hipMemcpyAsync(&NM, outOff + NT, 8, hipMemcpyDeviceToHost, st));
    LRA_HIP_CHECK(ctx, hipStreamSynchronize(st));
    char* wm = (char*)lra_ensure(ctx, 29, sz(NM + 1, 4) * 2 + 1024);
    if (!wm) return LRA_ERR_NOMEM;
    oq = (uint32_t*)take(wm, NM + 1, 4); ot = (uint32_t*)take(wm, NM + 1, 4);
    fa.oq = oq; fa.ot = ot;
    lra_time_begin(ctx, "rsc_filter");
    hipLaunchKernelGGL(av_filter<true>, dim3(gt), dim3(64), 0, st, fa);
    lra_time_end(ctx);
  } else {
    LRA_HIP_CHECK(ctx, hipMemsetAsync(outOff, 0, 16, st));
  }
  out->n_matches = NM; out->d_match_q = oq; out->d_match_t = ot;
  out->d_task_q_lo = a.qLo; out->d_task_q_hi = a.qHi; out->d_task_t_lo = a.tLo; out->d_task_t_hi = a.tHi;
  f.oq = oq; f.ot = ot;
  lra_time_begin(ctx, "rsc_filter");
  hipLaunchKernelGGL(rsc_match_off, dim3((unsigned)((NF + 2 + 255) / 256)), dim3(256), 0, st, f);
  hipLaunchKernelGGL(rsc_finish, dim3((unsigned)slots), dim3(64), 0, st, f);
  lra_time_end(ctx);
  LRA_HIP_CHECK(ctx, hipStreamSynchronize(st));
  LRA_HIP_CHECK(ctx, hipGetLastError());
  return LRA_OK;
}
```

lra_amd/csrc/std_sort.h:

```cpp
#pragma once
#include <stdint.h>

namespace lra_std_sort {

#define LRA_SS_FN __host__ __device__ __forceinline__

template <class T>
struct Ptr {
  typedef T value_type;
  T* v;
  template <class I> LRA_SS_FN T get(I i) const { return v[i]; }
  template <class I> LRA_SS_FN void set(I i, T x) const { v[i] = x; }
};
template <class P>
struct Pairs {
  struct value_type { uint64_t k; P p; };
  uint64_t* k; P* p;
  template <class I> LRA_SS_FN value_type get(I i) const { return value_type{k[i], p[i]}; }
  template <class I> LRA_SS_FN void set(I i, value_type x) const { k[i] = x.k; p[i] = x.p; }
};

template <class S, class I>
LRA_SS_FN void iter_swap(S s, I a, I b) { const typename S::value_type t = s.get(a); s.set(a, s.get(b)); s.set(b, t); }

template <class S, class I, class Less>
LRA_SS_FN void adjust_heap(S s, I first, I hole, I len, typename S::value_type val, const Less& lt) {
  const I top = hole;
  I child = hole;
  while (child < (len - 1) / 2) {
    child = 2 * (child + 1);
    if (lt(s.get(first + child), s.get(first + child - 1))) child--;
    s.set(first + hole, s.get(first + child));
    hole = child;
  }
  if ((len & 1) == 0 && child == (len - 2) / 2) {
    child = 2 * (child + 1);
    s.set(first + hole, s.get(first + child - 1));
    hole = child - 1;
  }
  I parent = (hole - 1) / 2;
  while (hole > top && lt(s.get(first + parent), val)) { s.set(first + hole, s.get(first + parent)); hole = parent; parent = (hole - 1) / 2; }
  s.set(first + hole, val);
}

template <class S, class I, class Less>
LRA_SS_FN void heap_sort(S s, I first, I last, const Less& lt) {
  const I len = last - first;
  if (len < 2) return;
  for (I parent = (len - 2) / 2;; parent--) { adjust_heap(s, first, parent, len, s.get(first + parent), lt); if (parent == 0) break; }
  while (last - first > 1) { --last; const typename S::value_type val = s.get(last); s.set(last, s.get(first)); adjust_heap(s, first, (I)0, last - first, val, lt); }
}

template <class S, class I, class Less>
LRA_SS_FN void move_median_to_first(S s, I first, I last, const Less& lt) {
  const I a = first + 1, b = first + (last - first) / 2, c = last - 1;
  const typename S::value_type va = s.get(a), vb = s.get(b), vc = s.get(c);
  if (lt(va, vb)) iter_swap(s, first, lt(vb, vc) ? b : lt(va, vc) ? c : a);
  else iter_swap(s, first, lt(va, vc) ? a : lt(vb, vc) ? c : b);
}

template <class S, class I, class Less>
LRA_SS_FN I unguarded_partition(S s, I first, I last, const Less& lt) {
  const typename S::value_type pv = s.get(first);
  I f = first + 1, l = last;
  while (true) {
    while (lt(s.get(f), pv)) ++f;
    --l;
    while (lt(pv, s.get(l))) --l;
    if (!(f < l)) return f;
    iter_swap(s, f, l);
    ++f;
  }
}

template <class S, class I, class Less>
LRA_SS_FN void unguarded_linear_insert(S s, I last, const Less& lt) {
  const typename S::value_type val = s.get(last);
  I next = last - 1;
  while (lt(val, s.get(next))) { s.set(last, s.get(next)); last = next; --next; }
  s.set(last, val);
}

template <class S, class I, class Less>
LRA_SS_FN void insertion_sort(S s, I first, I last, const Less& lt) {
  for (I i = first + 1; i < last; ++i) {
    const typename S::value_type val = s.get(i);
    I j = i;
    while (j > first && lt(val, s.get(j - 1))) { s.set(j, s.get(j - 1)); --j; }
    s.set(j, val);
  }
}

template <int DEPTH = 64, class S, class Less>
LRA_SS_FN void std_sort(S s, long n, const Less& lt) {
  if (n < 2) return;
  long stF[DEPTH], stL[DEPTH]; int stD[DEPTH];
  stF[0] = 0; stL[0] = n; stD[0] = 2 * (63 - __builtin_clzll((unsigned long long)n));
  int sp = 1;
  while (sp > 0) {
    --sp;
    const long first = stF[sp]; long last = stL[sp]; int depth = stD[sp];
    while (last - first > 16) {
      if (depth == 0) { heap_sort(s, first, last, lt); break; }
      --depth;
      move_median_to_first(s, first, last, lt);
      const long cut = unguarded_partition(s, first, last, lt);
      stF[sp] = cut; stL[sp] = last; stD[sp] = depth; sp++;
      last = cut;
    }
  }
  if (n > 16) {
    insertion_sort(s, 0L, 16L, lt);
    for (long i = 16; i < n; ++i) unguarded_linear_insert(s, i, lt);
  } else insertion_sort(s, 0L, n, lt);
}
template <int DEPTH = 64, class T, class Less>
LRA_SS_FN void std_sort(T* v, long n, const Less& lt) { std_sort<DEPTH>(Ptr<T>{v}, n, lt); }

#undef LRA_SS_FN

}
```

Measured before the change: 1.138.

## Move per-chain walks from one thread to one wavefront with LDS staging

Three kernels (me_trim, bt_apply, rsc_tasks) change from one thread per group or slot to one 64-lane wavefront per group or slot. Filtering, bounding-box reductions, break detection and binary searches become wave-parallel via ballot and shuffle reductions. me_trim packs its sort keys into LDS and sorts them on lane 0 with a shared-memory stack. The goal is to remove the serial per-thread walks and the load imbalance they cause, at the cost of more blocks, LDS pressure, idle lanes during the single-lane sort, and fallback serial paths for groups larger than the caps.

```diff
diff --git a/lra_amd/csrc/chain_walks.h b/lra_amd/csrc/chain_walks.h
--- /dev/null
+++ b/lra_amd/csrc/chain_walks.h
@@ -0,0 +1,28 @@
+#pragma once
+#include <hip/hip_runtime.h>
+#include <stdint.h>
+
+namespace lra_walks {
+
+constexpr int RSC_CAP = 1536;
+constexpr int ME_CAP = 1024;
+
+__device__ __forceinline__ uint32_t wave_min_u32(uint32_t v) { for (int o = 32; o; o >>= 1) v = min(v, (uint32_t)__shfl_xor((int)v, o)); return v; }
+__device__ __forceinline__ uint32_t wave_max_u32(uint32_t v) { for (int o = 32; o; o >>= 1) v = max(v, (uint32_t)__shfl_xor((int)v, o)); return v; }
+__device__ __forceinline__ int64_t wave_min_i64(int64_t v) { for (int o = 32; o; o >>= 1) v = min(v, (int64_t)__shfl_xor((long long)v, o)); return v; }
+__device__ __forceinline__ int64_t wave_max_i64(int64_t v) { for (int o = 32; o; o >>= 1) v = max(v, (int64_t)__shfl_xor((long long)v, o)); return v; }
+
+__device__ __forceinline__ long wave_lower_bound(const uint64_t* a, long n, uint64_t key, int lane) {
+  long lo = 0, hi = n;
+  while (hi > lo) {
+    const long step = (hi - lo + 63) / 64;
+    const long p = lo + (long)lane * step;
+    const int c = __popcll(__ballot(p < hi && a[p] < key));
+    if (c == 0) return lo;
+    const long nlo = lo + (long)(c - 1) * step + 1, nhi = lo + (long)c * step;
+    lo = nlo; hi = min(hi, nhi);
+  }
+  return lo;
+}
+
+}
diff --git a/lra_amd/csrc/merge_extend.hip b/lra_amd/csrc/merge_extend.hip
--- a/lra_amd/csrc/merge_extend.hip
+++ b/lra_amd/csrc/merge_extend.hip
@@ -1,9 +1,12 @@
 #include "common.h"
 #include "scan.h"
 #include "std_sort.h"
+#include "chain_walks.h"
 #include <rocprim/rocprim.hpp>
 
 namespace {
+
+using namespace lra_walks;
 
 struct MeArgs {
   uint64_t n_slots; int numAln; int K;
@@ -123,19 +126,12 @@
   }
 };
 
-__global__ void me_trim(uint64_t ng, const uint64_t* __restrict__ anchorOff, uint32_t* aq, uint32_t* at, int32_t* alen, const int32_t* __restrict__ gstrand,
-                        uint64_t* scratch, int minLen) {
-  const uint64_t g = (uint64_t)blockIdx.x * blockDim.x + threadIdx.x;
-  if (g >= ng) return;
-  const uint64_t b = anchorOff[g];
-  const uint32_t n = (uint32_t)(anchorOff[g + 1] - b);
-  uint32_t* Q = aq + b; uint32_t* T = at + b; int32_t* L = alen + b;
-  uint64_t* idx = scratch + b;
-  const int S = gstrand ? gstrand[g] : 0;
+template <class St>
+__device__ void me_trim_lane(uint32_t n, uint32_t* Q, uint32_t* T, int32_t* L, uint64_t* idx, int S, int minLen, St& stack) {
   uint32_t m = 0;
   for (uint32_t i = 0; i < n; i++) if (L[i] >= minLen) idx[m++] = i;
   LongLess lt{Q, T, L, S};
-  lra_std_sort::std_sort(idx, (long)m, lt);
+  lra_std_sort::std_sort_on(lra_std_sort::Ptr<uint64_t>{idx}, (long)m, lt, stack);
   for (uint32_t ln = 1; ln < m; ln++) {
     const uint32_t prev = (uint32_t)idx[ln - 1], cur = (uint32_t)idx[ln];
     int overlap_r = 0, overlap_g = 0;
@@ -149,6 +145,70 @@
       const int overlap = max(overlap_r, overlap_g);
       if (S == 1) Q[prev] += (uint32_t)(overlap + 1);
       L[prev] -= overlap + 1;
+    }
+  }
+}
+
+struct KeyLess {
+  template <class V> __device__ bool operator()(const V& x, const V& y) const { return x.k < y.k; }
+};
+
+__global__ void __launch_bounds__(64) me_trim(uint64_t ng, const uint64_t* __restrict__ anchorOff, uint32_t* aq, uint32_t* at, int32_t* alen,
+                                              const int32_t* __restrict__ gstrand, uint64_t* scratch, int minLen) {
+  __shared__ uint64_t sKey[ME_CAP];
+  __shared__ uint32_t sIdx[ME_CAP];
+  __shared__ int32_t sLen[ME_CAP];
+  __shared__ uint16_t sPos[ME_CAP];
+  __shared__ lra_std_sort::Stack<64> sStack;
+  const uint64_t g = blockIdx.x;
+  const int lane = threadIdx.x;
+  const uint64_t b = anchorOff[g];
+  const uint32_t n = (uint32_t)(anchorOff[g + 1] - b);
+  uint32_t* Q = aq + b; uint32_t* T = at + b; int32_t* L = alen + b;
+  const int S = gstrand ? gstrand[g] : 0;
+  uint32_t m = 0;
+  for (uint32_t base = 0; base < n; base += 4 * 64) {
+    int32_t l[4];
+#pragma unroll
+    for (int u = 0; u < 4; u++) { const uint32_t i = base + 64 * u + lane; l[u] = i < n ? L[i] : 0; }
+#pragma unroll
+    for (int u = 0; u < 4; u++) {
+      const uint32_t i = base + 64 * u + lane;
+      const bool isLong = i < n && l[u] >= minLen;
+      const uint64_t longs = __ballot(isLong);
+      const uint32_t k = m + (uint32_t)__popcll(longs & ((1ull << lane) - 1));
+      if (isLong && k < (uint32_t)ME_CAP) { sIdx[k] = i; sLen[k] = l[u]; }
+      m += (uint32_t)__popcll(longs);
+    }
+  }
+  if (m > (uint32_t)ME_CAP) { if (lane == 0) me_trim_lane(n, Q, T, L, scratch + b, S, minLen, sStack); return; }
+  if (m < 2) return;
+  __syncthreads();
+  for (uint32_t k = lane; k < m; k += 64) {
+    const uint32_t i = sIdx[k], q = Q[i], t = T[i];
+    sKey[k] = ((uint64_t)(S == 0 ? q : ~(q + (uint32_t)sLen[k])) << 32) | t;
+    sPos[k] = (uint16_t)k;
+  }
+  __syncthreads();
+  if (lane == 0) lra_std_sort::std_sort_on(lra_std_sort::Pairs<uint16_t>{sKey, sPos}, (long)m, KeyLess(), sStack);
+  __syncthreads();
+  for (uint32_t ln = 1 + lane; ln < m; ln += 64) {
+    const uint64_t kp = sKey[ln - 1], kc = sKey[ln];
+    const uint32_t pp = sPos[ln - 1], pc = sPos[ln];
+    const uint32_t Lp = (uint32_t)sLen[pp], Lc = (uint32_t)sLen[pc], Tp = (uint32_t)kp, Tc = (uint32_t)kc;
+    const uint32_t Qp = S == 0 ? (uint32_t)(kp >> 32) : ~(uint32_t)(kp >> 32) - Lp, Qc = S == 0 ? (uint32_t)(kc >> 32) : ~(uint32_t)(kc >> 32) - Lc;
+    int overlap_r = 0, overlap_g = 0;
+    if (S == 0) {
+      if (Qc < Qp + Lp && Qc >= Qp + Lp - 30u) overlap_r = (int)(Qp + Lp - Qc);
+    } else {
+      if (Qc + Lc > Qp && Qc + Lc <= Qp + 30u) overlap_r = (int)(Qc + Lc - Qp);
+    }
+    if (Tc < Tp + Lp && Tc >= Tp + Lp - 30u) overlap_g = (int)(Tp + Lp - Tc);
+    if (overlap_r > 0 || overlap_g > 0) {
+      const int overlap = max(overlap_r, overlap_g);
+      const uint32_t prev = sIdx[pp];
+      if (S == 1) Q[prev] = Qp + (uint32_t)(overlap + 1);
+      L[prev] = (int32_t)Lp - (overlap + 1);
     }
   }
 }
@@ -243,7 +303,7 @@
   a.aq = (uint32_t*)take(wa, NA + 1, 4); a.at = (uint32_t*)take(wa, NA + 1, 4); a.alen = (int32_t*)take(wa, NA + 1, 4);
   lra_time_begin(ctx, "merge_extend");
   hipLaunchKernelGGL(me_concat, dim3((unsigned)std::min<uint64_t>(NG, (uint64_t)ctx->num_cu * 32)), dim3(64), 0, st, NG, a);
-  hipLaunchKernelGGL(me_trim, dim3((unsigned)((NG + 63) / 64)), dim3(64), 0, st, NG, (const uint64_t*)anchorOff, a.aq, a.at, a.alen, (const int32_t*)a.gstrand, a.scratch, 40);
+  hipLaunchKernelGGL(me_trim, dim3((unsigned)NG), dim3(64), 0, st, NG, (const uint64_t*)anchorOff, a.aq, a.at, a.alen, (const int32_t*)a.gstrand, a.scratch, 40);
   hipLaunchKernelGGL(me_iota, dim3((unsigned)((NG + 256) / 256)), dim3(256), 0, st, NG, iota);
   lra_time_end(ctx);
   LRA_HIP_CHECK(ctx, hipStreamSynchronize(st));
@@ -261,7 +321,7 @@
   uint64_t* scratch = (uint64_t*)lra_scratch(ctx, 2, (n_anchors + 1) * 8);
   if (!scratch) return LRA_ERR_NOMEM;
   lra_time_begin(ctx, "merge_extend");
-  hipLaunchKernelGGL(me_trim, dim3((unsigned)((n_lists + 63) / 64)), dim3(64), 0, ctx->stream, n_lists, d_off, d_q, d_t, d_len, (const int32_t*)nullptr, scratch, 50);
+  hipLaunchKernelGGL(me_trim, dim3((unsigned)n_lists), dim3(64), 0, ctx->stream, n_lists, d_off, d_q, d_t, d_len, (const int32_t*)nullptr, scratch, 50);
   lra_time_end(ctx);
   LRA_HIP_CHECK(ctx, hipStreamSynchronize(ctx->stream));
   LRA_HIP_CHECK(ctx, hipGetLastError());
@@ -276,7 +336,7 @@
   uint64_t* scratch = (uint64_t*)lra_scratch(ctx, 2, (n_anchors + 1) * 8);
   if (!scratch) return LRA_ERR_NOMEM;
   lra_time_begin(ctx, "merge_extend");
-  hipLaunchKernelGGL(me_trim, dim3((unsigned)((n_clusters + 63) / 64)), dim3(64), 0, ctx->stream, n_clusters, d_off, d_q, d_t, d_len, d_strand, scratch, 40);
+  hipLaunchKernelGGL(me_trim, dim3((unsigned)n_clusters), dim3(64), 0, ctx->stream, n_clusters, d_off, d_q, d_t, d_len, d_strand, scratch, 40);
   lra_time_end(ctx);
   LRA_HIP_CHECK(ctx, hipStreamSynchronize(ctx->stream));
   LRA_HIP_CHECK(ctx, hipGetLastError());
diff --git a/lra_amd/csrc/refine_btwn.hip b/lra_amd/csrc/refine_btwn.hip
--- a/lra_amd/csrc/refine_btwn.hip
+++ b/lra_amd/csrc/refine_btwn.hip
@@ -1,10 +1,13 @@
 #include "common.h"
 #include "scan.h"
+#include "chain_walks.h"
 #include <rocprim/rocprim.hpp>
 #include <algorithm>
 #include <vector>
 
 namespace {
+
+using namespace lra_walks;
 
 constexpr uint32_t NONE = 0xFFFFFFFFu;
 
@@ -149,26 +152,34 @@
   if (i < n) out[i] = ((uint64_t)q[i] << 32) | t[i];
 }
 
-__device__ void append_seg(const BtArgs& a, uint64_t x, uint64_t off, uint32_t len) {
+struct PairBox { uint32_t qs, qe, ts, te; };
+
+__device__ __forceinline__ PairBox wave_pair_box(const BtArgs& a, uint64_t off, uint32_t len, int lane) {
+  PairBox b = {0xFFFFFFFFu, 0u, 0xFFFFFFFFu, 0u};
+  for (uint32_t i = lane; i < len; i += 64) {
+    const uint64_t v = a.pool[off + i];
+    const uint32_t q = (uint32_t)(v >> 32), t = (uint32_t)v;
+    b.qs = min(b.qs, q); b.qe = max(b.qe, q + (uint32_t)a.K); b.ts = min(b.ts, t); b.te = max(b.te, t + (uint32_t)a.K);
+  }
+  b.qs = wave_min_u32(b.qs); b.qe = wave_max_u32(b.qe); b.ts = wave_min_u32(b.ts); b.te = wave_max_u32(b.te);
+  return b;
+}
+
+__device__ void append_seg(const BtArgs& a, uint64_t x, uint64_t off, uint32_t len, const PairBox& b) {
   if (len == 0) return;
   const uint32_t id = atomicAdd(a.segCount, 1u);
   if (id >= a.segCap) { *a.overflow = 1; return; }
   a.segs[id].off = off; a.segs[id].len = len; a.segs[id].next = NONE;
   if (a.segHead[x] == NONE) a.segHead[x] = id; else a.segs[a.segTail[x]].next = id;
   a.segTail[x] = id;
-  uint32_t qs = a.box[4 * x], qe = a.box[4 * x + 1], ts = a.box[4 * x + 2], te = a.box[4 * x + 3];
-  for (uint32_t i = 0; i < len; i++) {
-    const uint64_t v = a.pool[off + i];
-    const uint32_t q = (uint32_t)(v >> 32), t = (uint32_t)v;
-    qs = min(qs, q); qe = max(qe, q + (uint32_t)a.K); ts = min(ts, t); te = max(te, t + (uint32_t)a.K);
-  }
-  a.box[4 * x] = qs; a.box[4 * x + 1] = qe; a.box[4 * x + 2] = ts; a.box[4 * x + 3] = te;
+  a.box[4 * x] = min(a.box[4 * x], b.qs); a.box[4 * x + 1] = max(a.box[4 * x + 1], b.qe);
+  a.box[4 * x + 2] = min(a.box[4 * x + 2], b.ts); a.box[4 * x + 3] = max(a.box[4 * x + 3], b.te);
   a.cnt[x] += len;
 }
 
-__global__ void bt_apply(BtArgs a) {
-  const uint64_t s = (uint64_t)blockIdx.x * blockDim.x + threadIdx.x;
-  if (s >= a.n_slots) return;
+__global__ void __launch_bounds__(64) bt_apply(BtArgs a) {
+  const uint64_t s = blockIdx.x;
+  const int lane = threadIdx.x;
   for (int j = 0; j < 2; j++) {
     const uint64_t i = 2 * s + j;
     if (!a.need[i]) continue;
@@ -179,36 +190,45 @@
     const float eff = ((float)n) / (float)a.mSpan[i];
     const uint64_t x = cs + a.mX[i], xp = cs + a.mXp[i];
     if (n == 0) continue;
-    if (a.mKind[i] == 1) { append_seg(a, x, a.poolU + p0, n); a.rspace[x] = 1; continue; }
-    if (eff >= a.sparse2) { append_seg(a, x, a.poolU + p0, n); a.rspace[x] = 1; continue; }
+    if (a.mKind[i] == 1 || eff >= a.sparse2) {
+      const PairBox b = wave_pair_box(a, a.poolU + p0, n, lane);
+      if (lane == 0) { append_seg(a, x, a.poolU + p0, n, b); a.rspace[x] = 1; }
+      continue;
+    }
     if (a.mTwo[i]) continue;
     const uint64_t* S = a.pool + a.poolS + p0;
     const int st = a.mSt[i];
     uint32_t start = 0;
-    while (start < n) {
-      uint32_t end = start + 1;
-      while (end < n) {
-        const long long dq = llabs((long long)(uint32_t)(S[end] >> 32) - (long long)(uint32_t)(S[end - 1] >> 32));
-        const long long dt = llabs((long long)(uint32_t)S[end] - (long long)(uint32_t)S[end - 1]);
-        if (min(dq, dt) <= 200) end++; else break;
+    for (uint64_t base = 1; base <= n; base += 64) {
+      const uint64_t e = base + lane;
+      bool brk = e == n;
+      if (e < n) {
+        const uint64_t v = S[e], u = S[e - 1];
+        const long long dq = llabs((long long)(uint32_t)(v >> 32) - (long long)(uint32_t)(u >> 32));
+        const long long dt = llabs((long long)(uint32_t)v - (long long)(uint32_t)u);
+        brk = min(dq, dt) > 200;
       }
-      if (end - start >= 4) {
-        uint32_t qS = (uint32_t)(S[start] >> 32), qE = qS + a.K, tS = (uint32_t)S[start], tE = tS + a.K;
-        for (uint32_t k = start + 1; k < end; k++) {
-          const uint32_t q = (uint32_t)(S[k] >> 32), t = (uint32_t)S[k];
-          tE = max(tE, t + (uint32_t)a.K); tS = min(tS, t); qE = max(qE, q + (uint32_t)a.K); qS = min(qS, q);
+      uint64_t ends = __ballot(brk);
+      while (ends) {
+        const uint32_t end = (uint32_t)base + (uint32_t)__builtin_ctzll(ends);
+        ends &= ends - 1;
+        if (end - start >= 4) {
+          const PairBox b = wave_pair_box(a, a.poolS + p0 + start, end - start, lane);
+          if (lane == 0) {
+            const uint32_t qS = b.qs, qE = b.qe, tS = b.ts, tE = b.te;
+            const uint32_t cqe = a.box[4 * x + 1], cts = a.box[4 * x + 2], cte = a.box[4 * x + 3];
+            const uint32_t pqs = a.box[4 * xp], pts = a.box[4 * xp + 2], pte = a.box[4 * xp + 3];
+            int qd = qS >= cqe ? (int)(qS - cqe) : 0, td;
+            if (st == 0) td = tS >= cte ? (int)(tS - cte) : 0; else td = cts >= tE ? (int)(cts - tE) : 0;
+            const int dist_cur = max(qd, td);
+            qd = pqs >= qE ? (int)(pqs - qE) : 0;
+            if (st == 0) td = pts >= tE ? (int)(pts - tE) : 0; else td = tS >= pte ? (int)(tS - pte) : 0;
+            const int dist_prev = max(qd, td);
+            append_seg(a, dist_cur <= dist_prev ? x : xp, a.poolS + p0 + start, end - start, b);
+          }
         }
-        const uint32_t cqe = a.box[4 * x + 1], cts = a.box[4 * x + 2], cte = a.box[4 * x + 3];
-        const uint32_t pqs = a.box[4 * xp], pts = a.box[4 * xp + 2], pte = a.box[4 * xp + 3];
-        int qd = qS >= cqe ? (int)(qS - cqe) : 0, td;
-        if (st == 0) td = tS >= cte ? (int)(tS - cte) : 0; else td = cts >= tE ? (int)(cts - tE) : 0;
-        const int dist_cur = max(qd, td);
-        qd = pqs >= qE ? (int)(pqs - qE) : 0;
-        if (st == 0) td = pts >= tE ? (int)(pts - tE) : 0; else td = tS >= pte ? (int)(tS - pte) : 0;
-        const int dist_prev = max(qd, td);
-        append_seg(a, dist_cur <= dist_prev ? x : xp, a.poolS + p0 + start, end - start);
+        start = end;
       }
-      start = end;
     }
   }
 }
@@ -367,7 +387,7 @@
       if (e != hipSuccess) return lra_set_err(ctx, LRA_ERR_HIP, "segmented sort: %s", hipGetErrorString(e));
     }
     lra_time_begin(ctx, "btwn_apply");
-    hipLaunchKernelGGL(bt_apply, dim3(gs), dim3(256), 0, st, a);
+    hipLaunchKernelGGL(bt_apply, dim3((unsigned)slots), dim3(64), 0, st, a);
     lra_time_end(ctx);
     poolUsed += 2 * nP;
   }
diff --git a/lra_amd/csrc/refine_splitchain.hip b/lra_amd/csrc/refine_splitchain.hip
--- a/lra_amd/csrc/refine_splitchain.hip
+++ b/lra_amd/csrc/refine_splitchain.hip
@@ -1,9 +1,12 @@
 #include "common.h"
 #include "append_values.h"
 #include "scan.h"
+#include "chain_walks.h"
 #include <vector>
 
 namespace {
+
+using namespace lra_walks;
 
 struct RscArgs {
   uint64_t n_slots; int numAln;
@@ -39,23 +42,14 @@
 }
 
 template <bool EMIT>
-__global__ void __launch_bounds__(64) rsc_tasks(RscArgs a) {
-  const uint64_t s = (uint64_t)blockIdx.x * blockDim.x + threadIdx.x;
-  if (s >= a.n_slots) return;
-  const uint64_t r = s / a.numAln;
-  if ((uint32_t)(s % a.numAln) >= a.nChains[r]) return;
-  const uint64_t cs = a.chainStart[s];
-  const uint32_t readLen = (uint32_t)(a.read_off[r + 1] - a.read_off[r]);
-  const long nWq = ((long)readLen + a.lwin - 1) / a.lwin;
-  const uint32_t nsp = a.spStatus[s] ? 0 : a.nSplit[s];
-  for (uint32_t k = 0; k < nsp; k++) {
-    const uint64_t x = cs + k;
+__device__ void rsc_split_walk(const RscArgs& a, uint64_t r, uint64_t cs, uint32_t readLen, long nWq, uint64_t x) {
+  {
     const int m = (int)a.spLen[x];
     uint32_t ntask = 0;
     uint64_t to = EMIT ? a.taskOff[x] : 0;
     if (!EMIT) { a.taskCnt[x] = 0; a.status[x] = 0; }
-    else if (a.status[x]) continue;
-    if (m == 0) continue;
+    else if (a.status[x]) return;
+    if (m == 0) return;
     const uint32_t* idx = a.spIdx + cs + a.spBeg[x];
     const uint32_t* ci = a.ciIdx + cs + a.ciBeg[x];
     const int nci = (int)a.ciLen[x];
@@ -69,7 +63,7 @@
     const uint32_t QStart = a.spBox[4 * x], QEnd = a.spBox[4 * x + 1], TStart = a.spBox[4 * x + 2], TEnd = a.spBox[4 * x + 3];
     bool ub = false;
     const int fi = header_find(a.pos, a.npos, TEnd, ub);
-    if (ub || fi + 1 >= a.npos) { if (!EMIT) a.status[x] = LRA_ST_OOB_SLOT; continue; }
+    if (ub || fi + 1 >= a.npos) { if (!EMIT) a.status[x] = LRA_ST_OOB_SLOT; return; }
     const uint32_t chromEndOffset = (uint32_t)a.pos[fi + 1];
     int64_t maxDN = (int64_t)tS(0) - (int64_t)qS(0), minDN = maxDN;
     if (!a.limitrefine)
@@ -78,7 +72,7 @@
     const uint32_t wts = (TStart >= chromOffset + (uint32_t)a.window) ? TStart - a.window : chromOffset;
     const uint32_t wte = (TEnd + (uint32_t)a.window < chromEndOffset) ? TEnd + a.window : chromEndOffset;
     const long ls = lookup_index(a.gSeqOff, (long)a.nWg + 1, wts, ub), le = lookup_index(a.gSeqOff, (long)a.nWg + 1, wte, ub);
-    if (ub) { if (!EMIT) a.status[x] = LRA_ST_OOB_SLOT; continue; }
+    if (ub) { if (!EMIT) a.status[x] = LRA_ST_OOB_SLOT; return; }
     const uint32_t qStart = Strand == 0 ? QStart : readLen - QEnd, qEnd = Strand == 0 ? QEnd : readLen - QStart;
     const uint64_t w0 = a.qWinOff[(Strand ? a.n_reads : 0) + r];
     int matchStart = 0, matchEnd = 0;
@@ -125,8 +119,153 @@
       }
     }
     (void)qE; (void)qStart; (void)qEnd;
-    if (bad) { if (!EMIT) { a.status[x] = LRA_ST_OOB_SLOT; a.taskCnt[x] = 0; } continue; }
+    if (bad) { if (!EMIT) { a.status[x] = LRA_ST_OOB_SLOT; a.taskCnt[x] = 0; } return; }
     if (!EMIT) a.taskCnt[x] = ntask;
+  }
+}
+
+__device__ int header_find_wave(const uint64_t* pos, int npos, uint64_t query, bool& ub, int lane) {
+  if (npos > 0 && query == pos[0]) return 0;
+  const int lo = (int)wave_lower_bound(pos, npos, query, lane);
+  if (lo == npos) { ub = true; return lo - 1; }
+  if (query == pos[lo]) return lo;
+  return lo - 1;
+}
+
+__device__ long lookup_index_wave(const uint64_t* so, long n, uint64_t pos, bool& ub, int lane) {
+  if (n == 0) return 0;
+  const long lo = wave_lower_bound(so, n, pos, lane);
+  if (lo == n) { ub = true; return lo - 1; }
+  if (so[lo] != pos) return lo - 1;
+  return lo;
+}
+
+template <bool LE>
+__device__ __forceinline__ int rsc_first_stop(const uint32_t* v, int m, int from, uint32_t bound, int lane) {
+  for (;;) {
+    const int i = from + lane;
+    const bool go = i < m && (LE ? v[i] <= bound : v[i] < bound);
+    const uint64_t stop = ~__ballot(go);
+    if (stop) return from + __builtin_ctzll(stop);
+    from += 64;
+  }
+}
+
+template <bool EMIT>
+__global__ void __launch_bounds__(64) rsc_tasks(RscArgs a) {
+  __shared__ uint32_t sT[RSC_CAP], sQ[RSC_CAP], sE[RSC_CAP];
+  const uint64_t s = blockIdx.x;
+  const int lane = threadIdx.x;
+  const uint64_t r = s / a.numAln;
+  if ((uint32_t)(s % a.numAln) >= a.nChains[r]) return;
+  const uint64_t cs = a.chainStart[s];
+  const uint32_t readLen = (uint32_t)(a.read_off[r + 1] - a.read_off[r]);
+  const long nWq = ((long)readLen + a.lwin - 1) / a.lwin;
+  const uint32_t nsp = a.spStatus[s] ? 0 : a.nSplit[s];
+  for (uint32_t k = 0; k < nsp; k++) {
+    const uint64_t x = cs + k;
+    const int m = (int)a.spLen[x];
+    if (m > RSC_CAP) { if (lane == 0) rsc_split_walk<EMIT>(a, r, cs, readLen, nWq, x); continue; }
+    uint32_t ntask = 0;
+    uint64_t to = EMIT ? a.taskOff[x] : 0;
+    if (!EMIT) { if (lane == 0) { a.taskCnt[x] = 0; a.status[x] = 0; } }
+    else if (a.status[x]) continue;
+    if (m == 0) continue;
+    const uint32_t* idx = a.spIdx + cs + a.spBeg[x];
+    const uint32_t* ci = a.ciIdx + cs + a.ciBeg[x];
+    const int nci = (int)a.ciLen[x];
+    const int Strand = a.spStrand[x];
+    const uint32_t chromOffset = (uint32_t)a.pos[a.spChrom[x]];
+    const uint32_t TStart = a.spBox[4 * x + 2], TEnd = a.spBox[4 * x + 3];
+    bool ub = false;
+    const int fi = header_find_wave(a.pos, a.npos, TEnd, ub, lane);
+    if (ub || fi + 1 >= a.npos) { if (!EMIT && lane == 0) a.status[x] = LRA_ST_OOB_SLOT; continue; }
+    const uint32_t chromEndOffset = (uint32_t)a.pos[fi + 1];
+    const uint32_t wts = (TStart >= chromOffset + (uint32_t)a.window) ? TStart - a.window : chromOffset;
+    const uint32_t wte = (TEnd + (uint32_t)a.window < chromEndOffset) ? TEnd + a.window : chromEndOffset;
+    const long ls = lookup_index_wave(a.gSeqOff, (long)a.nWg + 1, wts, ub, lane), le = lookup_index_wave(a.gSeqOff, (long)a.nWg + 1, wte, ub, lane);
+    if (ub) { if (!EMIT && lane == 0) a.status[x] = LRA_ST_OOB_SLOT; continue; }
+    __syncthreads();
+    for (int base = 0; base < m; base += 4 * 64) {
+      uint64_t p[4]; uint32_t c[4], t[4], q[4]; int32_t l[4]; uint8_t st[4]; bool flipped[4];
+#pragma unroll
+      for (int u = 0; u < 4; u++) p[u] = cs + a.fidx[cs + idx[min(base + 64 * u + lane, m - 1)]];
+#pragma unroll
+      for (int u = 0; u < 4; u++) { c[u] = a.ccl[p[u]]; t[u] = a.ct[p[u]]; q[u] = a.cq[p[u]]; l[u] = a.clen[p[u]]; st[u] = a.cstrand[p[u]]; flipped[u] = false; }
+      for (int j = 0; j < nci; j++) {
+        const uint32_t cj = ci[j];
+#pragma unroll
+        for (int u = 0; u < 4; u++) flipped[u] |= c[u] == cj;
+      }
+#pragma unroll
+      for (int u = 0; u < 4; u++) {
+        const int i = base + 64 * u + lane;
+        if (i < m) {
+          const uint32_t tS = flipped[u] ? t[u] - chromOffset : t[u];
+          const uint32_t qS = (st[u] == 1 && flipped[u]) ? readLen - (q[u] + (uint32_t)a.K) : q[u];
+          sT[i] = tS; sQ[i] = qS; sE[i] = qS + (uint32_t)l[u];
+        }
+      }
+    }
+    __syncthreads();
+    int64_t maxDN = (int64_t)sT[0] - (int64_t)sQ[0], minDN = maxDN;
+    if (!a.limitrefine) {
+      for (int db = lane; db < m; db += 64) { const int64_t d = (int64_t)sT[db] - (int64_t)sQ[db]; maxDN = max(maxDN, d); minDN = min(minDN, d); }
+      maxDN = wave_max_i64(maxDN); minDN = wave_min_i64(minDN);
+    }
+    const int64_t maxDiagNum = maxDN + 50, minDiagNum = minDN - 50;
+    const uint64_t w0 = a.qWinOff[(Strand ? a.n_reads : 0) + r];
+    int matchStart = 0, matchEnd = 0;
+    bool bad = false;
+    for (long lsi = ls; lsi <= le; lsi++) {
+      if (lsi + 1 > (long)a.nWg) continue;
+      const uint64_t g0 = a.gSeqOff[lsi], g1 = a.gSeqOff[lsi + 1];
+      if (g0 < chromOffset || g1 < chromOffset) continue;
+      const uint32_t gStart = (uint32_t)(g0 - chromOffset), gEnd = (uint32_t)(g1 - 1 - chromOffset);
+      if (gStart >= gEnd) continue;
+      matchStart = rsc_first_stop<true>(sT, m, matchStart, gStart, lane);
+      if (matchStart >= m) break;
+      matchEnd = rsc_first_stop<false>(sT, m, matchStart, gEnd, lane);
+      if (matchEnd == matchStart) continue;
+      uint32_t rs = 0xFFFFFFFFu, re = 0;
+      int64_t mm = INT64_MAX;
+      for (int mi = matchStart + lane; mi < matchEnd; mi += 64) {
+        const uint32_t q0 = sQ[mi];
+        rs = min(rs, q0); re = max(re, sE[mi]); mm = min(mm, (int64_t)sT[mi] - (int64_t)q0);
+      }
+      uint32_t readStart = wave_min_u32(rs), readEnd = max(sQ[matchEnd - 1], wave_max_u32(re));
+      int64_t miniMin = wave_min_i64(mm);
+      const int64_t miniMax = (int64_t)1 << 60;
+      if (readStart == readEnd) { if (lsi > ls && readStart > 0) readStart = 0; }
+      miniMin -= 100;
+      const uint32_t sow = 500;
+      if (lsi == ls) readStart = (readStart < sow) ? 0 : readStart - sow;
+      if (lsi == le) readEnd = (readEnd + sow > readLen) ? readLen : readEnd + sow;
+      if (readStart > readEnd) continue;
+      const uint32_t e2 = min(readEnd, readLen - 1);
+      const long qi0 = readStart == readLen ? nWq : (long)(readStart / (uint32_t)a.lwin);
+      const long qi1 = (long)(e2 / (uint32_t)a.lwin);
+      if (readStart > readLen) { bad = true; break; }
+      const long nq = qi1 - qi0 + 1;
+      if (nq <= 0) continue;
+      if (EMIT) {
+        const uint64_t tLo = a.gBnd[lsi], tHi = a.gBnd[lsi + 1];
+        for (long j = lane; j < nq; j += 64) {
+          const long qi = qi0 + j;
+          const uint64_t o = to + (uint64_t)j;
+          a.qLo[o] = a.qBnd[w0 + qi]; a.qHi[o] = a.qBnd[w0 + qi + 1];
+          a.tLo[o] = tLo; a.tHi[o] = tHi;
+          a.qAdd[o] = (uint32_t)min((long)readLen, qi * (long)a.lwin); a.tAdd[o] = gStart;
+          a.mx[o] = a.limitrefine ? miniMax : maxDiagNum; a.mn[o] = a.limitrefine ? miniMin : minDiagNum;
+        }
+        to += (uint64_t)nq;
+      }
+      ntask += (uint32_t)nq;
+    }
+    if (!EMIT && lane == 0) {
+      if (bad) { a.status[x] = LRA_ST_OOB_SLOT; a.taskCnt[x] = 0; }
+      else a.taskCnt[x] = ntask;
+    }
   }
 }
 
@@ -234,9 +373,8 @@
   LRA_HIP_CHECK(ctx, hipMemcpyAsync(dpos, h_chrom_pos, npos * 8, hipMemcpyHostToDevice, st));
   LRA_HIP_CHECK(ctx, hipMemsetAsync(a.taskCnt, 0, (NF + 2) * 4, st));
   LRA_HIP_CHECK(ctx, hipMemsetAsync(a.status, 0, (NF + 2) * 4, st));
-  const unsigned gs = (unsigned)((slots + 63) / 64);
   lra_time_begin(ctx, "rsc_tasks");
-  hipLaunchKernelGGL(rsc_tasks<false>, dim3(gs), dim3(64), 0, st, a);
+  hipLaunchKernelGGL(rsc_tasks<false>, dim3((unsigned)slots), dim3(64), 0, st, a);
   lra_time_end(ctx);
   { int rc = lra_exclusive_scan<uint32_t>(ctx, (long)NF + 1, a.taskCnt, taskOff); if (rc) return rc; }
   uint64_t NT = 0;
@@ -259,7 +397,7 @@
   uint32_t* oq = nullptr; uint32_t* ot = nullptr;
   if (NT > 0) {
     lra_time_begin(ctx, "rsc_tasks");
-    hipLaunchKernelGGL(rsc_tasks<true>, dim3(gs), dim3(64), 0, st, a);
+    hipLaunchKernelGGL(rsc_tasks<true>, dim3((unsigned)slots), dim3(64), 0, st, a);
     hipLaunchKernelGGL(rsc_task_box, dim3((unsigned)slots), dim3(64), 0, st, slots, ch->num_aln, ch->d_n_chains, ch->d_chain_start, sp->d_n_split, sp->d_status,
                        (const uint64_t*)taskOff, sp->d_sp_box, sp->d_sp_strand, sp->d_sp_chrom, (const uint64_t*)dpos, d_read_off, tbox);
     lra_time_end(ctx);
diff --git a/lra_amd/csrc/std_sort.h b/lra_amd/csrc/std_sort.h
--- a/lra_amd/csrc/std_sort.h
+++ b/lra_amd/csrc/std_sort.h
@@ -91,21 +91,22 @@
   }
 }
 
-template <int DEPTH = 64, class S, class Less>
-LRA_SS_FN void std_sort(S s, long n, const Less& lt) {
+template <int DEPTH>
+struct Stack { long f[DEPTH], l[DEPTH]; int d[DEPTH]; };
+template <class S, class Less, class St>
+LRA_SS_FN void std_sort_on(S s, long n, const Less& lt, St& st) {
   if (n < 2) return;
-  long stF[DEPTH], stL[DEPTH]; int stD[DEPTH];
-  stF[0] = 0; stL[0] = n; stD[0] = 2 * (63 - __builtin_clzll((unsigned long long)n));
+  st.f[0] = 0; st.l[0] = n; st.d[0] = 2 * (63 - __builtin_clzll((unsigned long long)n));
   int sp = 1;
   while (sp > 0) {
     --sp;
-    const long first = stF[sp]; long last = stL[sp]; int depth = stD[sp];
+    const long first = st.f[sp]; long last = st.l[sp]; int depth = st.d[sp];
     while (last - first > 16) {
       if (depth == 0) { heap_sort(s, first, last, lt); break; }
       --depth;
       move_median_to_first(s, first, last, lt);
       const long cut = unguarded_partition(s, first, last, lt);
-      stF[sp] = cut; stL[sp] = last; stD[sp] = depth; sp++;
+      st.f[sp] = cut; st.l[sp] = last; st.d[sp] = depth; sp++;
       last = cut;
     }
   }
@@ -114,6 +115,8 @@
     for (long i = 16; i < n; ++i) unguarded_linear_insert(s, i, lt);
   } else insertion_sort(s, 0L, n, lt);
 }
+template <int DEPTH = 64, class S, class Less>
+LRA_SS_FN void std_sort(S s, long n, const Less& lt) { Stack<DEPTH> st; std_sort_on(s, n, lt, st); }
 template <int DEPTH = 64, class T, class Less>
 LRA_SS_FN void std_sort(T* v, long n, const Less& lt) { std_sort<DEPTH>(Ptr<T>{v}, n, lt); }
 
```

Result: no change. 1.148 (median of 6 runs) (+0.9%).
